# leo19941227/Speech-Enhancement-by-S3PRL

Hardware: AMD Instinct MI355X
Metric: enhanced 10s utts/sec (higher is better)
Workload: dtype bf16; 1 GPU; configs[1]: TERA/Mockingjay upstream (6x768x12x3072, pretrain_sample.yaml) + TransformerSpecPredictionHead, evaluate()-style pass, 10 s @ 16 kHz; batch_per_gpu=32, global_batch=32, layers=6, frames=1001, parallelism=dp1 (utterance-sharded inference, no data-path collective), weights=seeded random, real sizes, ranks=single process, no process group

## Files before the change

include/se_amd.h:

```cpp
#ifndef SE_AMD_H_
#define SE_AMD_H_

#include <stddef.h>
#include <stdint.h>

#ifdef __cplusplus
extern "C" {
#endif

typedef enum se_status {
  SE_OK = 0,
  SE_ERR_INVALID = -1,
  SE_ERR_UNSUPPORTED = -2,
  SE_ERR_HIP = -3,
  SE_ERR_OOM = -4,
  SE_ERR_NO_DEVICE = -5
} se_status;

typedef enum se_act { SE_ACT_IDENTITY = 0, SE_ACT_RELU = 1, SE_ACT_SIGMOID = 2, SE_ACT_GELU = 3, SE_ACT_EXP = 4 } se_act;

const char* se_last_error(void);
const char* se_version(void);
int se_device_available(void);

typedef struct se_plan se_plan;

typedef struct se_geometry {
  int sample_rate;
  int win;
  int hop;
  int n_freq;
  int n_mels;
} se_geometry;

int se_plan_create(const se_geometry* geom, se_plan** out);
int se_plan_create_any(const se_geometry* geom, se_plan** out);
void se_plan_destroy(se_plan* plan);
int se_plan_n_fft(const se_plan* plan);
int se_plan_chunk_frames(const se_plan* plan, int inverse);
int se_plan_tables(const se_plan* plan, float* window, float* mel_fb);

int se_num_frames(const se_plan* plan, int n_samples);

int se_stft_f32(const se_plan* plan, const float* wavs, int B, int C, int T, int channel,
                float* power, float* phase, float* complx, float* mel, void* stream);
int se_stft2_f32(const se_plan* plan, const float* wavs, int B, int C, int T, int channel_a, float* power_a, float* phase_a, float* complx_a,
                 float* mel_a, int channel_b, float* power_b, float* phase_b, float* complx_b, float* mel_b, void* stream);

int se_stft_tphase_f32(const se_plan* plan, const float* wavs, int B, int C, int T, int channel_a, float* power_a, unsigned* tphase_a, float* mel_a,
                       int channel_b, float* power_b, unsigned* tphase_b, float* mel_b, void* stream);

size_t se_features_workspace_bytes(int B, int D, int F, int delta);
int se_features_f32(const float* raw, int raw_time_major, int B, int D, int F,
                    int apply_log, int delta, int cmvn, float eps,
                    float* out, void* workspace, size_t workspace_bytes, void* stream);
int se_features2_f32(const float* raw, int raw_time_major, int B, int D, int F,
                     int apply_log, int delta, int cmvn, float eps,
                     float* out, void* workspace, size_t workspace_bytes,
                     uint16_t* out_bf16_pad, int ld_pad, int32_t* valid_count, void* stream);

size_t se_features3_workspace_bytes(int B, int D, int delta);
size_t se_features3_colstats_workspace_bytes(int B, int D, int F, int delta);
int se_features3_f32(const float* raw, int raw_time_major, int B, int D, int F, int apply_log, int delta, int cmvn, float eps,
                     float* out, void* workspace, size_t workspace_bytes, uint16_t* out_bf16_pad, int ld_pad, int32_t* valid_count,
                     float* colstats_out, float colstats_eps, void* stream);

int se_istft_f32(const se_plan* plan, const float* power, const float* phase, int B, int F,
                 float linear_power, float* wav_out, int wav_stride,
                 const int64_t* lengths, float* sumsq_out, void* stream);

int se_istft_tphase_f32(const se_plan* plan, const float* power, const unsigned* tphase, int B, int F, int log_input,
                        float* wav_out, int wav_stride, const int64_t* lengths, float* sumsq_out,
                        const float* ref, int ref_stride, float* ref_sumsq_out, void* stream);

int se_masked_sumsq_f32(const float* x, int B, int T, int x_stride, const int64_t* lengths, float* sums, void* stream);

int se_dbnorm_f32(float* wav, int B, int T, int wav_stride, const int64_t* lengths,
                  const float* wav_sumsq, const float* ref_sumsq, float fixed_db, float eps, void* stream);

int se_dbnorm_bwd_f32(const float* wav_norm, const float* grad_out, int B, int T, int wav_stride, const int64_t* lengths,
                      const float* wav_sumsq, const float* ref_sumsq, float fixed_db, float eps, double* scratch, float* grad_wav,
                      void* stream);

int se_istft_bwd_f32(const se_plan* plan, const float* grad_wav, int wav_stride, const float* power, const float* phase,
                     const unsigned* tphase, int B, int F, float* grad_power, void* stream);
int se_istft_bwd_chunk_frames(const se_plan* plan);

size_t se_stft_bwd_workspace_bytes(const se_plan* plan, int B, int T);
int se_stft_bwd_f32(const se_plan* plan, const float* grad_power, const float* grad_complx, const float* complx, int B, int F, int T,
                    float* grad_wav, int wav_stride, void* workspace, size_t workspace_bytes, void* stream);
int se_stft_bwd_chunk(const se_plan* plan);

int se_length_masks_i64(const int64_t* lengths, int B, int max_len, int64_t* masks, void* stream);

size_t se_head_workspace_bytes(int B, int F, int D, int N);
int se_head_linear_f32(const float* feats, const float* W, const float* bias, const float* linears,
                       int B, int F, int D, int N, int act, int cmvn, float eps,
                       float* predicted, float* offset, void* workspace, size_t workspace_bytes, void* stream);

size_t se_head_w3_bytes(int N, int D);
int se_head_colstats_f32(const float* feats, int B, int F, int D, float eps, float* stats, void* stream);
int se_head_split_weights_f32(const float* W, int N, int D, uint16_t* W3, void* stream);
int se_head_linear_pre_f32(const float* feats, const uint16_t* W3, const float* bias, const float* linears, const float* stats,
                           int B, int F, int D, int N, int act, float* predicted, float* offset, void* stream);

size_t se_head_sisdr_scratch_doubles(int B, int F, int N);
int se_head_linear_sisdr_f32(const float* feats, const uint16_t* W3, const float* bias, const float* linears, const float* stats,
                             int B, int F, int D, int N, int act, float* predicted, float* offset,
                             const float* linear_tar, const int64_t* lengths, int len_div, float eps, double* scratch,
                             float* loss_b, double* sums_out, float* loss_out, void* stream);
int se_sisdr_head_mean_f32(const double* slab, int B, int F, int tile_rows, float eps, float* loss_b, double* sums_out, float* loss_out, void* stream);

int se_head_linear_bwd_f32(const float* feats, const float* linears, const float* offset, const float* grad_predicted,
                           const float* grad_offset, int B, int F, int D, int N, int act, int cmvn, float eps,
                           float* gW, float* gb, void* workspace, size_t workspace_bytes, void* stream);
size_t se_head_dx_workspace_bytes(int B, int F, int D, int N);
int se_head_linear_dx_f32(const float* feats, const float* linears, const float* offset, const float* grad_predicted,
                          const float* grad_offset, const float* W, int B, int F, int D, int N, int act, int cmvn, float eps,
                          float* dx, void* workspace, size_t workspace_bytes, void* stream);

int se_l1_masked_f32(const float* log_pred, const float* linear_tar, const int64_t* frame_lengths,
                     int B, int F, int K, float eps, double* sums, float* grad, void* stream);
size_t se_l1_scratch_doubles(int B);
int se_l1_masked_loss_f32(const float* log_pred, const float* linear_tar, const int64_t* lengths, int len_div, int B, int F, int K, float eps,
                          double* scratch3, double* sums_out, float* loss_out, float* grad, void* stream);

typedef struct se_encoder se_encoder;

typedef struct se_encoder_config {
  int input_dim;
  int hidden;
  int layers;
  int heads;
  int intermediate;
  float ln_eps;
  int spec_out;
  int fused_ln_min_rows;
} se_encoder_config;

typedef struct se_encoder_weights {
  const float *in_w, *in_b, *in_ln_w, *in_ln_b;
  const float* const *q_w, * const *q_b, * const *k_w, * const *k_b, * const *v_w, * const *v_b;
  const float* const *ao_w, * const *ao_b, * const *aln_w, * const *aln_b;
  const float* const *ff1_w, * const *ff1_b, * const *ff2_w, * const *ff2_b, * const *oln_w, * const *oln_b;
  const float *sh_dense_w, *sh_dense_b, *sh_ln_w, *sh_ln_b, *sh_out_w, *sh_out_b;
} se_encoder_weights;

int se_encoder_create(const se_encoder_config* cfg, const se_encoder_weights* w, se_encoder** out);
void se_encoder_destroy(se_encoder* enc);
size_t se_encoder_workspace_bytes(const se_encoder* enc, int B, int T);

int se_encoder_fwd_bf16(const se_encoder* enc, const float* feats, const int32_t* lengths, int B, int T,
                        float* hidden, void* workspace, size_t workspace_bytes, void* stream);
int se_encoder_fwd2_bf16(const se_encoder* enc, const float* feats, const uint16_t* feats_bf16_pad, const int32_t* lengths, int B, int T,
                         float* hidden, void* workspace, size_t workspace_bytes, void* stream);

int se_spechead_fwd_bf16(const se_encoder* enc, const float* hidden, int B, int T, int log_target, int act, float eps,
                         float* predicted, float* log_predicted, float* raw,
                         void* workspace, size_t workspace_bytes, void* stream);
int se_spechead_fwd2_bf16(const se_encoder* enc, const float* hidden, int B, int T, int log_target, int act, float eps,
                          float* predicted, float* log_predicted, float* raw,
                          void* workspace, size_t workspace_bytes, int x_bf_valid, void* stream);

int se_valid_lengths_i32(const float* feats, int B, int T, int D, int32_t* lengths, void* stream);

int se_gemm_bf16(const uint16_t* A, int lda, const uint16_t* W, int ldw, const float* bias,
                 const float* residual_f32, int M, int N, int K, int act,
                 uint16_t* out_bf16, float* out_f32, int ldc, void* stream);
int se_gemm_res_ln_bf16(const uint16_t* A, int lda, const uint16_t* W, int ldw, const float* bias, const float* residual_f32,
                        const float* ln_w, const float* ln_b, float eps, int M, int N, int K,
                        float* out_f32, uint16_t* out_bf16, void* stream);
int se_mhsa_fwd_bf16(const uint16_t* qkv, const int32_t* lengths, int B, int T, int heads, uint16_t* ctx, void* stream);
int se_mhsa_fwd_prescaled_bf16(const uint16_t* qkv, const int32_t* lengths, int B, int T, int heads, uint16_t* ctx, void* stream);
int se_mhsa_fwd_prescaled_variant_bf16(const uint16_t* qkv, const int32_t* lengths, int B, int T, int heads, uint16_t* ctx, int variant, void* stream);
size_t se_gemm_res24_scratch_bytes(void);
size_t se_gemm_res24_lo_bytes(int M);
int se_gemm_res24_ln_bf16(const uint16_t* A, int lda, const uint16_t* W, int ldw, const float* bias, const uint16_t* res_hi, const uint8_t* res_lo,
                          const float* ln_w, const float* ln_b, float eps, int M, int N, int K, float* out_f32, uint16_t* out_bf16, uint8_t* out_lo,
                          int variant, void* scratch, void* stream);

int se_layernorm_f32(const float* x, const float* w, const float* b, int M, int H, float eps,
                     float* out_f32, uint16_t* out_bf16, void* stream);
int se_cast_f32_bf16(const float* x, size_t n, uint16_t* out, void* stream);

int se_gemm_f32(const float* A, long lda, const float* W, long ldw, int w_kmajor, const float* bias, const float* residual, int res_mod,
                int M, int N, int K, int act, float alpha, float* C, long ldc, int batch_outer, int batch_inner, long strideA_outer,
                long strideA_inner, long strideW_outer, long strideW_inner, long strideC_outer, long strideC_inner, void* stream);
int se_softmax_rows_f32(float* scores, const int32_t* lengths, int B, int heads, int T, void* stream);
int se_split3_bf16(const float* x, long ld, int rows, int cols, int Kp, int which, uint16_t* out, void* stream);

int se_gemm_x3out_bf16(const uint16_t* A, int lda, const uint16_t* W, int ldw, const float* bias, int M, int N, int K, int act,
                       uint16_t* out3, int Kp, void* stream);
int se_layernorm_x3_f32(const float* x, const float* w, const float* b, int M, int H, float eps, float* out_f32, uint16_t* out3, int Kp,
                        void* stream);
int se_mhsa_fwd_x3_split_f32(const float* qkv, const int32_t* lengths, int B, int T, int heads, uint16_t* ctx3, int Kp, void* stream);
int se_gemm_res_ln_x3_bf16(const uint16_t* A, int lda, const uint16_t* W, int ldw, const float* bias, const float* residual_f32, const float* ln_w,
                           const float* ln_b, float eps, int M, int N, int K, float* out_f32, uint16_t* out3, void* stream);
int se_mhsa_fwd_x3_f32(const float* qkv, const int32_t* lengths, int B, int T, int heads, float* ctx, void* stream);

int se_transpose_bf16(const uint16_t* in, int rows, int cols, int ld_in, uint16_t* out, int ld_out, void* stream);
int se_transpose_f32_bf16(const float* in, int rows, int cols, int ld_in, uint16_t* out, int ld_out, void* stream);
int se_wgrad_bf16(const uint16_t* dYt, const uint16_t* Xt, int Mp, int N, int K, int splits, float* dW, int accumulate,
                  void* workspace, size_t workspace_bytes, void* stream);
int se_wgrad_tn_bf16(const uint16_t* dY, int ldy, const uint16_t* X, int ldx, int M, int N, int K, int splits, float* dW,
                     int accumulate, void* workspace, size_t workspace_bytes, void* stream);
int se_wgrad_tn_slabs_bf16(const uint16_t* dY, int ldy, const uint16_t* X, int ldx, int M, int N, int K, int rows_per_slab,
                           float* slabs, void* stream);
int se_colsum_f32(const float* x, int rows, int cols, int ld, float* out, int accumulate, void* stream);
int se_colsum_groups(const void* x, int is_bf16, int groups, int rows, int cols, int ld, float* out, void* stream);
int se_layernorm_bwd_f32(const float* x_in, const float* dy, const float* w, int M, int H, float eps, int gelu_in,
                         float* dx, uint16_t* dx_bf16, float* dgamma, float* dbeta, int accumulate, void* stream);
int se_layernorm_bwd_groups_f32(const float* x_in, const float* dy, const float* w, int groups, int rows, int H, float eps, int gelu_in,
                                float* dx, uint16_t* dx_bf16, float* dgamma, float* dbeta, void* stream);
int se_gelu_layernorm_f32(const float* pre, const float* w, const float* b, int M, int H, float eps,
                          float* out_f32, uint16_t* out_bf16, void* stream);
int se_spec_epilogue_f32(const float* p, size_t n, int log_target, int act, float eps, float* predicted, float* log_predicted, void* stream);
int se_spec_epilogue_bwd_f32(const float* p, const float* d_pred, const float* d_logp, int M, int N, int ldp, int log_target,
                             int act, float eps, float* dp_f32, uint16_t* dp_bf16, void* stream);

int se_mhsa_fwd_lse_bf16(const uint16_t* qkv, const int32_t* lengths, int B, int T, int heads, uint16_t* ctx, float* lse,
                         float dropout_p, uint64_t seed, uint32_t site, void* stream);
int se_mhsa_bwd_bf16(const uint16_t* qkv, const uint16_t* ctx, const uint16_t* d_ctx, const float* lse, const int32_t* lengths,
                     int B, int T, int heads, uint16_t* dqkv, float* dvec, float dropout_p, uint64_t seed, uint32_t site, void* stream);
int se_gelu_bf16(const uint16_t* x, size_t n, uint16_t* y, void* stream);
int se_gelu_bwd_bf16(const uint16_t* dy, const uint16_t* x, size_t n, uint16_t* dx, void* stream);

typedef struct se_encoder_grads {
  float *in_w, *in_b, *in_ln_w, *in_ln_b;
  float* const *q_w, * const *q_b, * const *k_w, * const *k_b, * const *v_w, * const *v_b;
  float* const *ao_w, * const *ao_b, * const *aln_w, * const *aln_b;
  float* const *ff1_w, * const *ff1_b, * const *ff2_w, * const *ff2_b, * const *oln_w, * const *oln_b;
} se_encoder_grads;

int se_encoder_refresh_bf16(se_encoder* enc, const se_encoder_weights* w, void* stream);
size_t se_encoder_saved_bytes(const se_encoder* enc, int B, int T);
size_t se_encoder_train_workspace_bytes(const se_encoder* enc, int B, int T);
int se_encoder_fwd_train_bf16(const se_encoder* enc, const float* feats, const int32_t* lengths, int B, int T, float* hidden,
                              void* saved, size_t saved_bytes, void* workspace, size_t workspace_bytes, float dropout_p, uint64_t seed,
                              void* stream);
int se_encoder_bwd_bf16(const se_encoder* enc, const int32_t* lengths, int B, int T, const float* d_hidden, const void* saved,
                        size_t saved_bytes, const se_encoder_grads* grads, void* workspace, size_t workspace_bytes, float dropout_p,
                        uint64_t seed, void* stream);
int se_encoder_bwd_cb_bf16(const se_encoder* enc, const int32_t* lengths, int B, int T, const float* d_hidden, const void* saved,
                           size_t saved_bytes, const se_encoder_grads* g, void* workspace, size_t workspace_bytes, float dropout_p,
                           uint64_t seed, void (*layer_done)(int layer, void* user), void* user, void* stream);

int se_multi_sumsq_f32(const float* const* grads, const uint64_t* sizes, int n_tensors, double* sumsq, void* stream);
int se_bertadam_step_f32(float* const* params, const float* const* grads, float* const* m, float* const* v, const uint64_t* sizes,
                         const float* weight_decay, int n_tensors, const double* sumsq, double lr_t, double b1, double b2, double e,
                         double max_grad_norm, double global_max_norm, void* stream);
int se_multi_copy_f32(float* const* dsts, const float* const* srcs, const uint64_t* sizes, int n_tensors, void* stream);

int se_mix_f32(const float* speech, int ld_s, const int64_t* len_s, const float* noise, int ld_n, const int64_t* len_n,
               const int64_t* off_n, const float* snr_db, int B, int T_out, int normalize, float target_level_db, float eps,
               float* wavs, double* sums, void* stream);
int se_sisdr_f32(const float* src, const float* tar, int ld, const int64_t* lengths, int B, float eps, double* sums, float* sisdr,
                 void* stream);
int se_sisdr_grad_f32(const float* src, const float* tar, int ld, const int64_t* lengths, int B, float eps, const double* sums,
                      float grad_scale, float* grad, void* stream);

typedef struct se_stoi_plan se_stoi_plan;
int se_stoi_plan_create(int sample_rate, se_stoi_plan** out);
void se_stoi_plan_destroy(se_stoi_plan* plan);
size_t se_stoi_workspace_bytes(const se_stoi_plan* plan, int B, int T);
int se_stoi_f32(const se_stoi_plan* plan, const float* clean, const float* processed, int ld, const int64_t* lengths, int B, int T, int extended,
                float* stoi_out, int32_t* kept_out, float* tob_out, void* workspace, size_t workspace_bytes, void* stream);
size_t se_stoi_grad_workspace_bytes(const se_stoi_plan* plan, int B, int T);
int se_stoi_grad_f32(const se_stoi_plan* plan, const float* clean, const float* processed, int ld, const int64_t* lengths, int B, int T,
                     int extended, float grad_scale, float* stoi_out, float* grad , void* workspace, size_t workspace_bytes,
                     void* stream);

int se_lstm_fwd_bf16(const uint16_t* w_hh, const float* xproj, int B, int T, int ndir, uint16_t* h_out, float* gates_out, float* c_out,
                     void* stream);
int se_lstm_bwd_bf16(const uint16_t* w_hh_t, const float* gates, const float* c_saved, const float* dh_out, int ld_dh, int B, int T,
                     int ndir, uint16_t* dgates_out, void* stream);
int se_colsum_bf16(const uint16_t* x, int rows, int cols, int ld, float* out, void* stream);

int se_sisdr_spec_f32(const float* predicted, const float* linear_tar, const int64_t* frame_lengths, int B, int F, int N, float eps,
                      float grad_scale, double* scratch, float* loss_b, float* grad, void* stream);

size_t se_sisdr_spec_loss_scratch_doubles(int B, int F, int N);
int se_sisdr_spec_loss_f32(const float* predicted, const float* linear_tar, const int64_t* lengths, int len_div, int B, int F, int N, float eps,
                           double* scratch, float* loss_b, double* sums_out, float* loss_out, void* stream);

int se_wsd_energy_f32(const float* linear_tar, int B, int F, int N, float* energy, float* energy_max, void* stream);
int se_wsd_f32(const float* linear_inp, const float* offset, const float* linear_tar, const int64_t* frame_lengths, const float* energy,
               const float* energy_max, int B, int F, int N, float alpha, float db_interval, float eps, float grad_scale, double* sums,
               float* grad, void* stream);

size_t se_specdist_scratch_doubles(int B, int F, int K);
int se_specdist_loss_f32(const float* power_pred, const float* power_tar, const int64_t* lengths, int hop, int B, int F, int K, float clamp,
                         double* scratch, float* loss_b, void* stream);
int se_specdist_grad_f32(const float* power_pred, const float* power_tar, const int64_t* lengths, int hop, int B, int F, int K, float clamp,
                         const double* scratch, float grad_scale, float* grad_power_pred, void* stream);

int se_prof_enable(int on);
int se_prof_reset(void);
int se_prof_read(int kind, double* total_ms, double* total_work, long long* launches);

#ifdef __cplusplus
}
#endif
#endif
```

speech-enhancement-by-s3prl_amd/_lib.py:

```python
import ctypes
import os
from ctypes import POINTER, c_char_p, c_double, c_float, c_int, c_int32, c_int64, c_size_t, c_uint16, c_void_p

import torch

from . import checkpoint as _checkpoint

_HERE = os.path.dirname(os.path.abspath(__file__))
LIB_PATH = os.environ.get('SE_AMD_LIB') or os.path.join(_HERE, 'libse_amd.so')

SE_ACT = {'Identity': 0, 'ReLU': 1, 'Sigmoid': 2, 'GELU': 3, 'Exp': 4}


class SEError(RuntimeError):
    pass


class Geometry(ctypes.Structure):
    _fields_ = [('sample_rate', c_int), ('win', c_int), ('hop', c_int), ('n_freq', c_int), ('n_mels', c_int)]


class EncoderConfig(ctypes.Structure):
    _fields_ = [('input_dim', c_int), ('hidden', c_int), ('layers', c_int), ('heads', c_int), ('intermediate', c_int),
                ('ln_eps', c_float), ('spec_out', c_int), ('fused_ln_min_rows', c_int)]


_FP = POINTER(c_float)
_FPP = POINTER(_FP)


class EncoderWeights(ctypes.Structure):
    _fields_ = ([(n, _FP) for n in ('in_w', 'in_b', 'in_ln_w', 'in_ln_b')] +
                [(n, _FPP) for n in ('q_w', 'q_b', 'k_w', 'k_b', 'v_w', 'v_b', 'ao_w', 'ao_b', 'aln_w', 'aln_b',
                                     'ff1_w', 'ff1_b', 'ff2_w', 'ff2_b', 'oln_w', 'oln_b')] +
                [(n, _FP) for n in ('sh_dense_w', 'sh_dense_b', 'sh_ln_w', 'sh_ln_b', 'sh_out_w', 'sh_out_b')])


class EncoderGrads(ctypes.Structure):
    _fields_ = ([(n, _FP) for n in ('in_w', 'in_b', 'in_ln_w', 'in_ln_b')] +
                [(n, _FPP) for n in ('q_w', 'q_b', 'k_w', 'k_b', 'v_w', 'v_b', 'ao_w', 'ao_b', 'aln_w', 'aln_b',
                                     'ff1_w', 'ff1_b', 'ff2_w', 'ff2_b', 'oln_w', 'oln_b')])


_P = c_void_p
LAYER_DONE_CB = ctypes.CFUNCTYPE(None, c_int, c_void_p)
SIGNATURES = {
    'se_last_error': (c_char_p, []),
    'se_version': (c_char_p, []),
    'se_device_available': (c_int, []),
    'se_plan_create': (c_int, [POINTER(Geometry), POINTER(_P)]),
    'se_plan_create_any': (c_int, [POINTER(Geometry), POINTER(_P)]),
    'se_plan_destroy': (None, [_P]),
    'se_plan_n_fft': (c_int, [_P]),
    'se_plan_chunk_frames': (c_int, [_P, c_int]),
    'se_plan_tables': (c_int, [_P, _P, _P]),
    'se_num_frames': (c_int, [_P, c_int]),
    'se_stft_f32': (c_int, [_P, _P, c_int, c_int, c_int, c_int, _P, _P, _P, _P, _P]),
    'se_stft2_f32': (c_int, [_P, _P, c_int, c_int, c_int, c_int, _P, _P, _P, _P, c_int, _P, _P, _P, _P, _P]),
    'se_stft_tphase_f32': (c_int, [_P, _P, c_int, c_int, c_int, c_int, _P, _P, _P, c_int, _P, _P, _P, _P]),
    'se_istft_tphase_f32': (c_int, [_P, _P, _P, c_int, c_int, c_int, _P, c_int, _P, _P, _P, c_int, _P, _P]),
    'se_features_workspace_bytes': (c_size_t, [c_int, c_int, c_int, c_int]),
    'se_features_f32': (c_int, [_P, c_int, c_int, c_int, c_int, c_int, c_int, c_int, c_float, _P, _P, c_size_t, _P]),
    'se_features2_f32': (c_int, [_P, c_int, c_int, c_int, c_int, c_int, c_int, c_int, c_float, _P, _P, c_size_t, _P, c_int, _P, _P]),
    'se_features3_workspace_bytes': (c_size_t, [c_int, c_int, c_int]),
    'se_features3_colstats_workspace_bytes': (c_size_t, [c_int, c_int, c_int, c_int]),
    'se_features3_f32': (c_int, [_P, c_int, c_int, c_int, c_int, c_int, c_int, c_int, c_float, _P, _P, c_size_t, _P, c_int, _P, _P, c_float, _P]),
    'se_istft_f32': (c_int, [_P, _P, _P, c_int, c_int, c_float, _P, c_int, _P, _P, _P]),
    'se_masked_sumsq_f32': (c_int, [_P, c_int, c_int, c_int, _P, _P, _P]),
    'se_dbnorm_f32': (c_int, [_P, c_int, c_int, c_int, _P, _P, _P, c_float, c_float, _P]),
    'se_dbnorm_bwd_f32': (c_int, [_P, _P, c_int, c_int, c_int, _P, _P, _P, c_float, c_float, _P, _P, _P]),
    'se_istft_bwd_f32': (c_int, [_P, _P, c_int, _P, _P, _P, c_int, c_int, _P, _P]),
    'se_istft_bwd_chunk_frames': (c_int, [_P]),
    'se_stft_bwd_workspace_bytes': (c_size_t, [_P, c_int, c_int]),
    'se_stft_bwd_f32': (c_int, [_P, _P, _P, _P, c_int, c_int, c_int, _P, c_int, _P, c_size_t, _P]),
    'se_stft_bwd_chunk': (c_int, [_P]),
    'se_length_masks_i64': (c_int, [_P, c_int, c_int, _P, _P]),
    'se_head_workspace_bytes': (c_size_t, [c_int, c_int, c_int, c_int]),
    'se_head_linear_f32': (c_int, [_P, _P, _P, _P, c_int, c_int, c_int, c_int, c_int, c_int, c_float, _P, _P, _P, c_size_t, _P]),
    'se_head_colstats_f32': (c_int, [_P, c_int, c_int, c_int, c_float, _P, _P]),
    'se_head_w3_bytes': (c_size_t, [c_int, c_int]),
    'se_head_split_weights_f32': (c_int, [_P, c_int, c_int, _P, _P]),
    'se_head_linear_pre_f32': (c_int, [_P, _P, _P, _P, _P, c_int, c_int, c_int, c_int, c_int, _P, _P, _P]),
    'se_head_sisdr_scratch_doubles': (c_size_t, [c_int, c_int, c_int]),
    'se_head_linear_sisdr_f32': (c_int, [_P, _P, _P, _P, _P, c_int, c_int, c_int, c_int, c_int, _P, _P, _P, _P, c_int, c_float, _P, _P, _P, _P, _P]),
    'se_sisdr_head_mean_f32': (c_int, [_P, c_int, c_int, c_int, c_float, _P, _P, _P, _P]),
    'se_head_linear_bwd_f32': (c_int, [_P, _P, _P, _P, _P, c_int, c_int, c_int, c_int, c_int, c_int, c_float, _P, _P, _P, c_size_t, _P]),
    'se_head_dx_workspace_bytes': (c_size_t, [c_int, c_int, c_int, c_int]),
    'se_head_linear_dx_f32': (c_int, [_P, _P, _P, _P, _P, _P, c_int, c_int, c_int, c_int, c_int, c_int, c_float, _P, _P, c_size_t, _P]),
    'se_l1_masked_f32': (c_int, [_P, _P, _P, c_int, c_int, c_int, c_float, _P, _P, _P]),
    'se_l1_scratch_doubles': (c_size_t, [c_int]),
    'se_l1_masked_loss_f32': (c_int, [_P, _P, _P, c_int, c_int, c_int, c_int, c_float, _P, _P, _P, _P, _P]),
    'se_encoder_create': (c_int, [POINTER(EncoderConfig), POINTER(EncoderWeights), POINTER(_P)]),
    'se_encoder_destroy': (None, [_P]),
    'se_encoder_workspace_bytes': (c_size_t, [_P, c_int, c_int]),
    'se_encoder_fwd_bf16': (c_int, [_P, _P, _P, c_int, c_int, _P, _P, c_size_t, _P]),
    'se_encoder_fwd2_bf16': (c_int, [_P, _P, _P, _P, c_int, c_int, _P, _P, c_size_t, _P]),
    'se_spechead_fwd_bf16': (c_int, [_P, _P, c_int, c_int, c_int, c_int, c_float, _P, _P, _P, _P, c_size_t, _P]),
    'se_spechead_fwd2_bf16': (c_int, [_P, _P, c_int, c_int, c_int, c_int, c_float, _P, _P, _P, _P, c_size_t, c_int, _P]),
    'se_valid_lengths_i32': (c_int, [_P, c_int, c_int, c_int, _P, _P]),
    'se_gemm_bf16': (c_int, [_P, c_int, _P, c_int, _P, _P, c_int, c_int, c_int, c_int, _P, _P, c_int, _P]),
    'se_gemm_res_ln_bf16': (c_int, [_P, c_int, _P, c_int, _P, _P, _P, _P, c_float, c_int, c_int, c_int, _P, _P, _P]),
    'se_gemm_res24_scratch_bytes': (c_size_t, []),
    'se_gemm_res24_lo_bytes': (c_size_t, [c_int]),
    'se_gemm_res24_ln_bf16': (c_int, [_P, c_int, _P, c_int, _P, _P, _P, _P, _P, c_float, c_int, c_int, c_int, _P, _P, _P, c_int, _P, _P]),
    'se_mhsa_fwd_bf16': (c_int, [_P, _P, c_int, c_int, c_int, _P, _P]),
    'se_mhsa_fwd_prescaled_bf16': (c_int, [_P, _P, c_int, c_int, c_int, _P, _P]),
    'se_mhsa_fwd_prescaled_variant_bf16': (c_int, [_P, _P, c_int, c_int, c_int, _P, c_int, _P]),
    'se_layernorm_f32': (c_int, [_P, _P, _P, c_int, c_int, c_float, _P, _P, _P]),
    'se_cast_f32_bf16': (c_int, [_P, c_size_t, _P, _P]),
    'se_gemm_f32': (c_int, [_P, ctypes.c_long, _P, ctypes.c_long, c_int, _P, _P, c_int, c_int, c_int, c_int, c_int, c_float, _P, ctypes.c_long, c_int, c_int,
                            ctypes.c_long, ctypes.c_long, ctypes.c_long, ctypes.c_long, ctypes.c_long, ctypes.c_long, _P]),
    'se_softmax_rows_f32': (c_int, [_P, _P, c_int, c_int, c_int, _P]),
    'se_split3_bf16': (c_int, [_P, ctypes.c_long, c_int, c_int, c_int, c_int, _P, _P]),
    'se_gemm_x3out_bf16': (c_int, [_P, c_int, _P, c_int, _P, c_int, c_int, c_int, c_int, _P, c_int, _P]),
    'se_layernorm_x3_f32': (c_int, [_P, _P, _P, c_int, c_int, c_float, _P, _P, c_int, _P]),
    'se_mhsa_fwd_x3_split_f32': (c_int, [_P, _P, c_int, c_int, c_int, _P, c_int, _P]),
    'se_gemm_res_ln_x3_bf16': (c_int, [_P, c_int, _P, c_int, _P, _P, _P, _P, c_float, c_int, c_int, c_int, _P, _P, _P]),
    'se_mhsa_fwd_x3_f32': (c_int, [_P, _P, c_int, c_int, c_int, _P, _P]),
    'se_transpose_bf16': (c_int, [_P, c_int, c_int, c_int, _P, c_int, _P]),
    'se_transpose_f32_bf16': (c_int, [_P, c_int, c_int, c_int, _P, c_int, _P]),
    'se_wgrad_bf16': (c_int, [_P, _P, c_int, c_int, c_int, c_int, _P, c_int, _P, c_size_t, _P]),
    'se_wgrad_tn_bf16': (c_int, [_P, c_int, _P, c_int, c_int, c_int, c_int, c_int, _P, c_int, _P, c_size_t, _P]),
    'se_wgrad_tn_slabs_bf16': (c_int, [_P, c_int, _P, c_int, c_int, c_int, c_int, c_int, _P, _P]),
    'se_colsum_f32': (c_int, [_P, c_int, c_int, c_int, _P, c_int, _P]),
    'se_colsum_groups': (c_int, [_P, c_int, c_int, c_int, c_int, c_int, _P, _P]),
    'se_layernorm_bwd_groups_f32': (c_int, [_P, _P, _P, c_int, c_int, c_int, c_float, c_int, _P, _P, _P, _P, _P]),
    'se_layernorm_bwd_f32': (c_int, [_P, _P, _P, c_int, c_int, c_float, c_int, _P, _P, _P, _P, c_int, _P]),
    'se_gelu_layernorm_f32': (c_int, [_P, _P, _P, c_int, c_int, c_float, _P, _P, _P]),
    'se_spec_epilogue_f32': (c_int, [_P, c_size_t, c_int, c_int, c_float, _P, _P, _P]),
    'se_spec_epilogue_bwd_f32': (c_int, [_P, _P, _P, c_int, c_int, c_int, c_int, c_int, c_float, _P, _P, _P]),
    'se_mhsa_fwd_lse_bf16': (c_int, [_P, _P, c_int, c_int, c_int, _P, _P, c_float, ctypes.c_uint64, ctypes.c_uint32, _P]),
    'se_mhsa_bwd_bf16': (c_int, [_P, _P, _P, _P, _P, c_int, c_int, c_int, _P, _P, c_float, ctypes.c_uint64, ctypes.c_uint32, _P]),
    'se_gelu_bf16': (c_int, [_P, c_size_t, _P, _P]),
    'se_gelu_bwd_bf16': (c_int, [_P, _P, c_size_t, _P, _P]),
    'se_encoder_refresh_bf16': (c_int, [_P, POINTER(EncoderWeights), _P]),
    'se_encoder_saved_bytes': (c_size_t, [_P, c_int, c_int]),
    'se_encoder_train_workspace_bytes': (c_size_t, [_P, c_int, c_int]),
    'se_encoder_fwd_train_bf16': (c_int, [_P, _P, _P, c_int, c_int, _P, _P, c_size_t, _P, c_size_t, c_float, ctypes.c_uint64, _P]),
    'se_encoder_bwd_bf16': (c_int, [_P, _P, c_int, c_int, _P, _P, c_size_t, POINTER(EncoderGrads), _P, c_size_t, c_float, ctypes.c_uint64, _P]),
    'se_encoder_bwd_cb_bf16': (c_int, [_P, _P, c_int, c_int, _P, _P, c_size_t, POINTER(EncoderGrads), _P, c_size_t, c_float, ctypes.c_uint64, _P, _P, _P]),
    'se_multi_sumsq_f32': (c_int, [_P, _P, c_int, _P, _P]),
    'se_bertadam_step_f32': (c_int, [_P, _P, _P, _P, _P, _P, c_int, _P, c_double, c_double, c_double, c_double, c_double, c_double, _P]),
    'se_multi_copy_f32': (c_int, [_P, _P, _P, c_int, _P]),
    'se_mix_f32': (c_int, [_P, c_int, _P, _P, c_int, _P, _P, _P, c_int, c_int, c_int, c_float, c_float, _P, _P, _P]),
    'se_sisdr_f32': (c_int, [_P, _P, c_int, _P, c_int, c_float, _P, _P, _P]),
    'se_sisdr_grad_f32': (c_int, [_P, _P, c_int, _P, c_int, c_float, _P, c_float, _P, _P]),
    'se_stoi_plan_create': (c_int, [c_int, POINTER(_P)]),
    'se_stoi_plan_destroy': (None, [_P]),
    'se_stoi_workspace_bytes': (c_size_t, [_P, c_int, c_int]),
    'se_stoi_f32': (c_int, [_P, _P, _P, c_int, _P, c_int, c_int, c_int, _P, _P, _P, _P, c_size_t, _P]),
    'se_stoi_grad_workspace_bytes': (c_size_t, [_P, c_int, c_int]),
    'se_stoi_grad_f32': (c_int, [_P, _P, _P, c_int, _P, c_int, c_int, c_int, c_float, _P, _P, _P, c_size_t, _P]),
    'se_lstm_fwd_bf16':(c_int, [_P, _P, c_int, c_int, c_int, _P, _P, _P, _P]),
    'se_lstm_bwd_bf16': (c_int, [_P, _P, _P, _P, c_int, c_int, c_int, c_int, _P, _P]),
    'se_colsum_bf16': (c_int, [_P, c_int, c_int, c_int, _P, _P]),
    'se_sisdr_spec_loss_scratch_doubles': (c_size_t, [c_int, c_int, c_int]),
    'se_sisdr_spec_loss_f32': (c_int, [_P, _P, _P, c_int, c_int, c_int, c_int, c_float, _P, _P, _P, _P, _P]),
    'se_sisdr_spec_f32': (c_int, [_P, _P, _P, c_int, c_int, c_int, c_float, c_float, _P, _P, _P, _P]),
    'se_wsd_energy_f32': (c_int, [_P, c_int, c_int, c_int, _P, _P, _P]),
    'se_wsd_f32': (c_int, [_P, _P, _P, _P, _P, _P, c_int, c_int, c_int, c_float, c_float, c_float, c_float, _P, _P, _P]),
    'se_specdist_scratch_doubles': (c_size_t, [c_int, c_int, c_int]),
    'se_specdist_loss_f32': (c_int, [_P, _P, _P, c_int, c_int, c_int, c_int, c_float, _P, _P, _P]),
    'se_specdist_grad_f32': (c_int, [_P, _P, _P, c_int, c_int, c_int, c_int, c_float, _P, c_float, _P, _P]),
    'se_prof_enable': (c_int, [c_int]),
    'se_prof_reset': (c_int, []),
    'se_prof_read': (c_int, [c_int, POINTER(c_double), POINTER(c_double), POINTER(ctypes.c_longlong)]),
}

_lib = None


def load():
    global _lib
    if _lib is not None:
        return _lib
    if not os.path.exists(LIB_PATH):
        raise SEError(f'{LIB_PATH} is missing: build it with `python speech-enhancement-by-s3prl_amd/build.py` '
                      '(or __graft_entry__.build()); the MI355X path has no CPU fallback')
    lib = ctypes.CDLL(LIB_PATH)
    for name, (res, args) in SIGNATURES.items():
        if not hasattr(lib, name) and os.environ.get('SE_AMD_ALLOW_PARTIAL') == '1':
            continue
        fn = getattr(lib, name)
        fn.restype = res
        fn.argtypes = args
    _lib = lib
    return lib


def last_error():
    return load().se_last_error().decode()


def check(status, what):
    if status != 0:
        raise SEError(f'{what} failed with status {status}: {last_error()}')


def ptr(t):
    if t is None:
        return None
    mat = getattr(t, 'materialize', None)
    if mat is not None:
        t = mat()
    if not t.is_cuda:
        raise SEError('libse_amd kernels take device tensors only (got a CPU tensor); there is no CPU fallback')
    if not t.is_contiguous():
        raise SEError('libse_amd kernels take contiguous tensors')
    return t.data_ptr()


def stream():
    return torch.cuda.current_stream().cuda_stream
```

speech-enhancement-by-s3prl_amd/csrc/encoder.hip:

```cpp
#include <math.h>
#include <stdlib.h>
#include <utility>
#include <vector>
#include "common.h"
#include "bf16.h"
#include "encoder_impl.h"

extern "C" int se_gemm2_splitk_launch(const uint16_t* A, int lda, const uint16_t* W, int ldw, int M, int N, int Kc, int splits,
                                      float* partials, void* stream);

namespace se {

template <int NV, int GELU_IN = 0>
__global__ __launch_bounds__(256) void layernorm_kernel(const float* __restrict__ x, const float* __restrict__ pe, int T,
                                                        const float* __restrict__ w, const float* __restrict__ b, int M, float eps,
                                                        float* __restrict__ out_f32, uint16_t* __restrict__ out_bf16) {
  constexpr int H = 256 * NV;
  const int lane = threadIdx.x & 63;
  const int row = blockIdx.x * 4 + (threadIdx.x >> 6);
  if (row >= M) return;
  const float* xr = x + (size_t)row * H;
  float4 v[NV];
#pragma unroll
  for (int i = 0; i < NV; ++i) v[i] = *reinterpret_cast<const float4*>(xr + (i * 64 + lane) * 4);
// ... 45 lines not shown
  const int lane = threadIdx.x & 63;
  const int row = blockIdx.x * 4 + (threadIdx.x >> 6);
  if (row >= M) return;
  float4 v[NV];
#pragma unroll
  for (int i = 0; i < NV; ++i) {
    const int c = (i * 64 + lane) * 4;
    const float4 bb = *reinterpret_cast<const float4*>(bias + c);
    const float4 rr = *reinterpret_cast<const float4*>(residual + (size_t)row * H + c);
    v[i] = make_float4(bb.x + rr.x, bb.y + rr.y, bb.z + rr.z, bb.w + rr.w);
    for (int sidx = 0; sidx < nslab; ++sidx) {
      const float4 p = *reinterpret_cast<const float4*>(partials + sidx * slab_stride + (size_t)row * H + c);
      v[i].x += p.x; v[i].y += p.y; v[i].z += p.z; v[i].w += p.w;
    }
  }
  float s = 0.f;
#pragma unroll
  for (int i = 0; i < NV; ++i) s += (v[i].x + v[i].y) + (v[i].z + v[i].w);
#pragma unroll
  for (int off = 32; off > 0; off >>= 1) s += __shfl_xor(s, off);
  const float mean = s * (1.0f / H);
  float q = 0.f;
#pragma unroll
  for (int i = 0; i < NV; ++i) {
    v[i].x -= mean; v[i].y -= mean; v[i].z -= mean; v[i].w -= mean;
    q += (v[i].x * v[i].x + v[i].y * v[i].y) + (v[i].z * v[i].z + v[i].w * v[i].w);
  }
#pragma unroll
  for (int off = 32; off > 0; off >>= 1) q += __shfl_xor(q, off);
  const float rstd = 1.0f / sqrtf(q * (1.0f / H) + eps);
#pragma unroll
  for (int i = 0; i < NV; ++i) {
    const int c = (i * 64 + lane) * 4;
    const float4 ww = *reinterpret_cast<const float4*>(w + c), bb = *reinterpret_cast<const float4*>(b + c);
    float4 y;
    y.x = ww.x * (v[i].x * rstd) + bb.x; y.y = ww.y * (v[i].y * rstd) + bb.y;
    y.z = ww.z * (v[i].z * rstd) + bb.z; y.w = ww.w * (v[i].w * rstd) + bb.w;
    if (out_f32) *reinterpret_cast<float4*>(out_f32 + (size_t)row * H + c) = y;
    if (out_bf16) *reinterpret_cast<uint2*>(out_bf16 + (size_t)row * H + c) = make_uint2(pack_bf16x2(y.x, y.y), pack_bf16x2(y.z, y.w));
  }
}

__global__ __launch_bounds__(256) void layernorm_generic_kernel(const float* __restrict__ x, const float* __restrict__ pe, int T,
                                                                const float* __restrict__ w, const float* __restrict__ b, int H, float eps,
                                                                float* __restrict__ out_f32, uint16_t* __restrict__ out_bf16) {
  __shared__ float red[4];
  const int row = blockIdx.x, tid = threadIdx.x;
  const float* xr = x + (size_t)row * H;
  const float* pr = pe ? pe + (size_t)(row % T) * H : nullptr;
  float s = 0.f;
  for (int c = tid; c < H; c += 256) s += xr[c] + (pr ? pr[c] : 0.f);
  for (int off = 32; off > 0; off >>= 1) s += __shfl_down(s, off);
  if ((tid & 63) == 0) red[tid >> 6] = s;
  __syncthreads();
  const float mean = (red[0] + red[1] + red[2] + red[3]) / (float)H;
  __syncthreads();
  float q = 0.f;
  for (int c = tid; c < H; c += 256) {
    const float d = xr[c] + (pr ? pr[c] : 0.f) - mean;
    q += d * d;
  }
  for (int off = 32; off > 0; off >>= 1) q += __shfl_down(q, off);
  if ((tid & 63) == 0) red[tid >> 6] = q;
  __syncthreads();
  const float rstd = 1.0f / sqrtf((red[0] + red[1] + red[2] + red[3]) / (float)H + eps);
  for (int c = tid; c < H; c += 256) {
    const float y = w[c] * ((xr[c] + (pr ? pr[c] : 0.f) - mean) * rstd) + b[c];
    if (out_f32) out_f32[(size_t)row * H + c] = y;
    if (out_bf16) out_bf16[(size_t)row * H + c] = f2bf(y);
  }
}

__global__ __launch_bounds__(256) void cast_pad_kernel(const float* __restrict__ x, size_t rows, int cols, int ld_out,
                                                       uint16_t* __restrict__ out) {
  const size_t n4 = rows * (size_t)(ld_out / 4);
  for (size_t i = blockIdx.x * (size_t)256 + threadIdx.x; i < n4; i += (size_t)gridDim.x * 256) {
    const size_t r = i / (ld_out / 4);
    const int c = (int)(i - r * (ld_out / 4)) * 4;
    float v0 = 0.f, v1 = 0.f, v2 = 0.f, v3 = 0.f;
    const float* xr = x + r * cols;
    if (c + 3 < cols && (cols % 4 == 0)) {
      const float4 t = *reinterpret_cast<const float4*>(xr + c);
      v0 = t.x; v1 = t.y; v2 = t.z; v3 = t.w;
    } else {
      if (c < cols) v0 = xr[c];
      if (c + 1 < cols) v1 = xr[c + 1];
      if (c + 2 < cols) v2 = xr[c + 2];
      if (c + 3 < cols) v3 = xr[c + 3];
    }
    *reinterpret_cast<uint2*>(out + r * ld_out + c) = make_uint2(pack_bf16x2(v0, v1), pack_bf16x2(v2, v3));
  }
}

__global__ __launch_bounds__(256) void valid_lengths_kernel(const float* __restrict__ feats, int T, int D, int32_t* __restrict__ lengths) {
  __shared__ int red[4];
  const int b = blockIdx.y, lane = threadIdx.x & 63, wv = threadIdx.x >> 6;
  int cnt = 0;
  for (int t = blockIdx.x * 4 + wv; t < T; t += gridDim.x * 4) {
    const float* fr = feats + ((size_t)b * T + t) * D;
    float s = 0.f;
    for (int d = lane; d < D; d += 64) s += fr[d];
#pragma unroll
    for (int off = 32; off > 0; off >>= 1) s += __shfl_xor(s, off);
    cnt += (s != 0.f) ? 1 : 0;
  }
  if (lane == 0) red[wv] = cnt;
  __syncthreads();
  if (threadIdx.x == 0) atomicAdd(&lengths[b], red[0] + red[1] + red[2] + red[3]);
}

__global__ __launch_bounds__(256) void spec_epilogue_kernel(const float* __restrict__ p, size_t n, int log_target, int act, float eps,
                                                            float* __restrict__ predicted, float* __restrict__ log_predicted) {
  for (size_t i = blockIdx.x * (size_t)256 + threadIdx.x; i < n; i += (size_t)gridDim.x * 256) {
    const float v = p[i];
    float pred, lp;
    if (log_target == 2) {
      lp = (act == SE_ACT_RELU) ? fmaxf(v, 0.f) : (act == SE_ACT_SIGMOID) ? 1.f / (1.f + expf(-v)) : v;
      pred = expf(lp);
    } else {
      if (log_target) {
        pred = expf(v);
        lp = v;
      } else {
        pred = v;
        lp = logf(v + eps);
      }
      if (act == SE_ACT_RELU) pred = fmaxf(pred, 0.f);
      else if (act == SE_ACT_SIGMOID) pred = 1.f / (1.f + expf(-pred));
    }
    if (predicted) predicted[i] = pred;
    if (log_predicted) log_predicted[i] = lp;
  }
}

__global__ __launch_bounds__(256) void spec_epilogue_rows_kernel(const float* __restrict__ p, int M, int N, int ld, int log_target, int act, float eps,
                                                                 float* __restrict__ predicted, float* __restrict__ log_predicted) {
  for (int r = blockIdx.x; r < M; r += gridDim.x) {
    for (int c = threadIdx.x; c < N; c += 256) {
      const float v = p[(size_t)r * ld + c];
      float pred, lp;
      if (log_target) {
        pred = expf(v);
        lp = v;
      } else {
        pred = v;
        lp = logf(v + eps);
      }
      if (act == SE_ACT_RELU) pred = fmaxf(pred, 0.f);
      else if (act == SE_ACT_SIGMOID) pred = 1.f / (1.f + expf(-pred));
      const size_t o = (size_t)r * N + c;
      if (predicted) predicted[o] = pred;
      if (log_predicted) log_predicted[o] = lp;
    }
  }
}

__global__ __launch_bounds__(256) void spec_epilogue_bwd_kernel(const float* __restrict__ p, const float* __restrict__ d_pred,
                                                                const float* __restrict__ d_logp, int M, int N, int ldp, int log_target,
                                                                int act, float eps, float* __restrict__ dp_f32, uint16_t* __restrict__ dp_bf16) {
  const size_t n = (size_t)M * ldp;
  for (size_t i = blockIdx.x * (size_t)256 + threadIdx.x; i < n; i += (size_t)gridDim.x * 256) {
    const size_t r = i / ldp;
    const int c = (int)(i - r * ldp);
    float g = 0.f;
    if (c < N) {
      const size_t j = r * N + c;
      const float v = p[j];
      const float gp = d_pred ? d_pred[j] : 0.f, gl = d_logp ? d_logp[j] : 0.f;
      if (log_target == 2) {
        const float sg = 1.f / (1.f + expf(-v));
        const float lp = (act == SE_ACT_RELU) ? fmaxf(v, 0.f) : (act == SE_ACT_SIGMOID) ? sg : v;
        const float da = (act == SE_ACT_RELU) ? (v > 0.f ? 1.f : 0.f) : (act == SE_ACT_SIGMOID) ? sg * (1.f - sg) : 1.f;
        g = (gl + gp * expf(lp)) * da;
      } else if (log_target) {
        const float e = expf(v);
        const float da = (act == SE_ACT_RELU) ? (e > 0.f ? 1.f : 0.f) : 1.f;
        g = gl + gp * da * e;
      } else {
        const float da = (act == SE_ACT_RELU) ? (v > 0.f ? 1.f : 0.f) : 1.f;
        g = gp * da + gl / (v + eps);
      }
      if (dp_f32) dp_f32[j] = g;
    }
    if (dp_bf16) dp_bf16[i] = f2bf(g);
  }
}

}

namespace se {
__global__ __launch_bounds__(256) void qkv_inf_kernel(const float* __restrict__ q_w, const float* __restrict__ q_b, const uint16_t* __restrict__ qkv_w,
                                                      const float* __restrict__ qkv_b, int H, uint16_t* __restrict__ w_inf, float* __restrict__ b_inf) {
  const size_t hh = (size_t)H * H;
  for (size_t e = (size_t)blockIdx.x * 256 + threadIdx.x; e < 3 * hh; e += (size_t)gridDim.x * 256)
    w_inf[e] = e < hh ? f2bf(q_w[e] * kQScale) : qkv_w[e];
  for (int e = blockIdx.x * 256 + threadIdx.x; e < 3 * H; e += gridDim.x * 256) b_inf[e] = e < H ? q_b[e] * kQScale : qkv_b[e];
}
int launch_qkv_inf(const float* q_w, const float* q_b, const uint16_t* qkv_w, const float* qkv_b, int H, uint16_t* qkv_w_inf, float* qkv_b_inf, hipStream_t st) {
  hipLaunchKernelGGL(qkv_inf_kernel, dim3(512), dim3(256), 0, st, q_w, q_b, qkv_w, qkv_b, H, qkv_w_inf, qkv_b_inf);
  SE_LAUNCH_CHECK();
  return SE_OK;
}
}

static inline uint16_t host_f2bf(float f) {
  uint32_t u;
  memcpy(&u, &f, 4);
  if ((u & 0x7fffffffu) > 0x7f800000u) return (uint16_t)((u >> 16) | 0x40);
  return (uint16_t)((u + 0x7fffu + ((u >> 16) & 1u)) >> 16);
}

int se::launch_cast_pad(const float* x, size_t rows, int cols, int ld_out, uint16_t* out, hipStream_t st) {
  const int grid = (int)std::min<size_t>((rows * (size_t)(ld_out / 4) + 255) / 256, 8192);
  hipLaunchKernelGGL(se::cast_pad_kernel, dim3(grid), dim3(256), 0, st, x, rows, cols, ld_out, out);
  SE_LAUNCH_CHECK();
  return SE_OK;
}

int se::launch_layernorm(const float* x, const float* pe, int T, const float* w, const float* b, int M, int H, float eps,
                         float* out_f32, uint16_t* out_bf16, hipStream_t st) {
  if (H == 768) {
    hipLaunchKernelGGL((se::layernorm_kernel<3>), dim3((M + 3) / 4), dim3(256), 0, st, x, pe, T, w, b, M, eps, out_f32, out_bf16);
  } else if (H == 256) {
    hipLaunchKernelGGL((se::layernorm_kernel<1>), dim3((M + 3) / 4), dim3(256), 0, st, x, pe, T, w, b, M, eps, out_f32, out_bf16);
  } else if (H == 512) {
    hipLaunchKernelGGL((se::layernorm_kernel<2>), dim3((M + 3) / 4), dim3(256), 0, st, x, pe, T, w, b, M, eps, out_f32, out_bf16);
  } else if (H == 1024) {
    hipLaunchKernelGGL((se::layernorm_kernel<4>), dim3((M + 3) / 4), dim3(256), 0, st, x, pe, T, w, b, M, eps, out_f32, out_bf16);
  } else {
    hipLaunchKernelGGL(se::layernorm_generic_kernel, dim3(M), dim3(256), 0, st, x, pe, T, w, b, H, eps, out_f32, out_bf16);
  }
  SE_LAUNCH_CHECK();
  return SE_OK;
}

extern "C" int se_layernorm_f32(const float* x, const float* w, const float* b, int M, int H, float eps,
                                float* out_f32, uint16_t* out_bf16, void* stream) {
  SE_REQUIRE(x && w && b && (out_f32 || out_bf16) && M > 0 && H > 0, "se_layernorm_f32: bad argument");
  return se::launch_layernorm(x, nullptr, 1, w, b, M, H, eps, out_f32, out_bf16, se::as_stream(stream));
}

extern "C" int se_gelu_layernorm_f32(const float* pre, const float* w, const float* b, int M, int H, float eps,
                                     float* out_f32, uint16_t* out_bf16, void* stream) {
  SE_REQUIRE(pre && w && b && (out_f32 || out_bf16) && M > 0, "se_gelu_layernorm_f32: bad argument");
  SE_REQUIRE(H == 768 || H == 256, "se_gelu_layernorm_f32: only H = 768 / 256 are built (got %d)", H);
  if (H == 768)
    hipLaunchKernelGGL((se::layernorm_kernel<3, 1>), dim3((M + 3) / 4), dim3(256), 0, se::as_stream(stream), pre, nullptr, 1, w, b, M, eps, out_f32, out_bf16);
  else
    hipLaunchKernelGGL((se::layernorm_kernel<1, 1>), dim3((M + 3) / 4), dim3(256), 0, se::as_stream(stream), pre, nullptr, 1, w, b, M, eps, out_f32, out_bf16);
  SE_LAUNCH_CHECK();
  return SE_OK;
}

extern "C" int se_spec_epilogue_f32(const float* p, size_t n, int log_target, int act, float eps, float* predicted, float* log_predicted,
                                    void* stream) {
  SE_REQUIRE(p && n > 0 && (predicted || log_predicted), "se_spec_epilogue_f32: bad argument");
  const int grid = (int)std::min<size_t>((n + 255) / 256, 8192);
  hipLaunchKernelGGL(se::spec_epilogue_kernel, dim3(grid), dim3(256), 0, se::as_stream(stream), p, n, log_target, act, eps, predicted, log_predicted);
  SE_LAUNCH_CHECK();
  return SE_OK;
}

extern "C" int se_spec_epilogue_bwd_f32(const float* p, const float* d_pred, const float* d_logp, int M, int N, int ldp, int log_target,
                                        int act, float eps, float* dp_f32, uint16_t* dp_bf16, void* stream) {
  SE_REQUIRE(p && (d_pred || d_logp) && (dp_f32 || dp_bf16) && M > 0 && N > 0 && ldp >= N, "se_spec_epilogue_bwd_f32: bad argument");
  SE_REQUIRE(act == SE_ACT_RELU || act == SE_ACT_IDENTITY || (log_target == 2 && act == SE_ACT_SIGMOID),
             "se_spec_epilogue_bwd_f32: activation must be ReLU or Identity (Sigmoid only with log_target 2)");
  const size_t n = (size_t)M * ldp;
  const int grid = (int)std::min<size_t>((n + 255) / 256, 8192);
  hipLaunchKernelGGL(se::spec_epilogue_bwd_kernel, dim3(grid), dim3(256), 0, se::as_stream(stream), p, d_pred, d_logp, M, N, ldp, log_target,
                     act, eps, dp_f32, dp_bf16);
  SE_LAUNCH_CHECK();
  return SE_OK;
}

extern "C" int se_cast_f32_bf16(const float* x, size_t n, uint16_t* out, void* stream) {
  SE_REQUIRE(x && out && n > 0 && n % 4 == 0, "se_cast_f32_bf16: n must be a positive multiple of 4");
  const size_t rows = n / 4;
  const int grid = (int)std::min<size_t>((rows + 255) / 256, 4096);
  hipLaunchKernelGGL(se::cast_pad_kernel, dim3(grid), dim3(256), 0, se::as_stream(stream), x, rows, 4, 4, out);
  SE_LAUNCH_CHECK();
  return SE_OK;
}

extern "C" int se_valid_lengths_i32(const float* feats, int B, int T, int D, int32_t* lengths, void* stream) {
  SE_REQUIRE(feats && lengths && B > 0 && T > 0 && D > 0, "se_valid_lengths_i32: bad argument");
  { const int zrc_ = se::zero_async(lengths, sizeof(int32_t) * B, se::as_stream(stream)); if (zrc_) return zrc_; }
  hipLaunchKernelGGL(se::valid_lengths_kernel, dim3(std::min(32, (T + 3) / 4), B), dim3(256), 0, se::as_stream(stream), feats, T, D, lengths);
  SE_LAUNCH_CHECK();
  return SE_OK;
}

extern "C" int se_encoder_create(const se_encoder_config* cfg, const se_encoder_weights* w, se_encoder** out) {
  SE_REQUIRE(cfg && w && out, "se_encoder_create: null argument");
  const int H = cfg->hidden, I = cfg->intermediate, L = cfg->layers, D = cfg->input_dim;
  if (cfg->heads <= 0 || H != cfg->heads * 64 || H % 64 != 0 || I % 64 != 0 || D <= 0 || D > se::kInPad || L <= 0) {
    se::set_error("se_encoder_create: unsupported config (hidden=%d heads=%d intermediate=%d input_dim=%d): head dim must be 64, "
                  "hidden/intermediate multiples of 64, input_dim <= %d", H, cfg->heads, I, D, se::kInPad);
    return SE_ERR_UNSUPPORTED;
  }
  int ndev = 0;
  if (hipGetDeviceCount(&ndev) != hipSuccess || ndev <= 0) {
    (void)hipGetLastError();
    se::set_error("se_encoder_create: no HIP device visible (no CPU fallback)");
    return SE_ERR_NO_DEVICE;
  }
  const bool has_head = cfg->spec_out > 0 && w->sh_dense_w;
  std::vector<char> host;
  auto reserve = [&](size_t bytes) {
    const size_t off = (host.size() + 255) & ~(size_t)255;
    host.resize(off + bytes, 0);
    return off;
  };
  auto put_f32 = [&](const float* src, size_t n) {
    const size_t off = reserve(n * 4);
    memcpy(host.data() + off, src, n * 4);
    return off;
  };
  auto put_bf16 = [&](const float* src, int rows, int cols, int ld) {
    const size_t off = reserve((size_t)rows * ld * 2);
    uint16_t* d = reinterpret_cast<uint16_t*>(host.data() + off);
    for (int r = 0; r < rows; ++r)
      for (int c = 0; c < cols; ++c) d[(size_t)r * ld + c] = host_f2bf(src[(size_t)r * cols + c]);
    return off;
  };
  struct Off { size_t in_w, in_b, in_ln_w, in_ln_b, pe; std::vector<std::vector<size_t>> l; size_t shd_w, shd_b, shl_w, shl_b, sho_w, sho_b; } o;
  o.in_w = put_bf16(w->in_w, H, D, se::kInPad);
  o.in_b = put_f32(w->in_b, H);
  o.in_ln_w = put_f32(w->in_ln_w, H);
  o.in_ln_b = put_f32(w->in_ln_b, H);
  {
    o.pe = reserve((size_t)se::kMaxPos * H * 4);
    float* pe = reinterpret_cast<float*>(host.data() + o.pe);
    for (int pos = 0; pos < se::kMaxPos; ++pos)
      for (int j = 0; j < H; ++j) {
        const double ang = (double)pos / pow(10000.0, 2.0 * (double)(j / 2) / (double)H);
        pe[(size_t)pos * H + j] = (float)((j & 1) ? cos(ang) : sin(ang));
      }
  }
  for (int i = 0; i < L; ++i) {
    std::vector<size_t> lo;
    {
      const size_t off = reserve((size_t)3 * H * H * 2);
      uint16_t* d = reinterpret_cast<uint16_t*>(host.data() + off);
      const float* srcs[3] = {w->q_w[i], w->k_w[i], w->v_w[i]};
      for (int p = 0; p < 3; ++p)
        for (size_t e = 0; e < (size_t)H * H; ++e) d[(size_t)p * H * H + e] = host_f2bf(srcs[p][e]);
      lo.push_back(off);
      const size_t boff = reserve((size_t)3 * H * 4);
      float* bd = reinterpret_cast<float*>(host.data() + boff);
      memcpy(bd, w->q_b[i], H * 4);
      memcpy(bd + H, w->k_b[i], H * 4);
      memcpy(bd + 2 * H, w->v_b[i], H * 4);
      lo.push_back(boff);
    }
    size_t inf_w, inf_b;
    {
      inf_w = reserve((size_t)3 * H * H * 2);
      uint16_t* d = reinterpret_cast<uint16_t*>(host.data() + inf_w);
      for (size_t e = 0; e < (size_t)H * H; ++e) d[e] = host_f2bf(w->q_w[i][e] * se::kQScale);
      for (size_t e = 0; e < (size_t)H * H; ++e) d[(size_t)H * H + e] = host_f2bf(w->k_w[i][e]);
      for (size_t e = 0; e < (size_t)H * H; ++e) d[(size_t)2 * H * H + e] = host_f2bf(w->v_w[i][e]);
      inf_b = reserve((size_t)3 * H * 4);
      float* bd = reinterpret_cast<float*>(host.data() + inf_b);
      for (int e = 0; e < H; ++e) bd[e] = w->q_b[i][e] * se::kQScale;
      memcpy(bd + H, w->k_b[i], H * 4);
      memcpy(bd + 2 * H, w->v_b[i], H * 4);
    }
    lo.push_back(put_bf16(w->ao_w[i], H, H, H));
    lo.push_back(put_f32(w->ao_b[i], H));
    lo.push_back(put_f32(w->aln_w[i], H));
    lo.push_back(put_f32(w->aln_b[i], H));
    lo.push_back(put_bf16(w->ff1_w[i], I, H, H));
    lo.push_back(put_f32(w->ff1_b[i], I));
    lo.push_back(put_bf16(w->ff2_w[i], H, I, I));
    lo.push_back(put_f32(w->ff2_b[i], H));
    lo.push_back(put_f32(w->oln_w[i], H));
    lo.push_back(put_f32(w->oln_b[i], H));
    lo.push_back(inf_w);
    lo.push_back(inf_b);
    o.l.push_back(lo);
  }
  if (has_head) {
    o.shd_w = put_bf16(w->sh_dense_w, H, H, H);
    o.shd_b = put_f32(w->sh_dense_b, H);
    o.shl_w = put_f32(w->sh_ln_w, H);
    o.shl_b = put_f32(w->sh_ln_b, H);
    o.sho_w = put_bf16(w->sh_out_w, cfg->spec_out, H, H);
    reserve((size_t)3 * H * 2);
    o.sho_b = put_f32(w->sh_out_b, cfg->spec_out);
    reserve(3 * 4);
  }
  se_encoder* e = new se_encoder();
  e->cfg = *cfg;
  if (!has_head) e->cfg.spec_out = 0;
  e->blob_bytes = host.size() + 256;
  hipError_t err = hipMalloc(&e->blob, e->blob_bytes);
  if (err != hipSuccess) {
    delete e;
    return se::hip_fail(err, "hipMalloc(encoder weights)", __FILE__, __LINE__);
  }
  err = hipMemcpy(e->blob, host.data(), host.size(), hipMemcpyHostToDevice);
  if (err != hipSuccess) {
    (void)hipFree(e->blob);
    delete e;
    return se::hip_fail(err, "hipMemcpy(encoder weights)", __FILE__, __LINE__);
  }
  char* base = reinterpret_cast<char*>(e->blob);
  e->in_w = (uint16_t*)(base + o.in_w);
  e->in_b = (float*)(base + o.in_b);
  e->in_ln_w = (float*)(base + o.in_ln_w);
// ... 3 lines not shown
    const auto& lo = o.l[i];
    se_encoder::Layer y;
    y.qkv_w = (uint16_t*)(base + lo[0]); y.qkv_b = (float*)(base + lo[1]);
    y.ao_w = (uint16_t*)(base + lo[2]); y.ao_b = (float*)(base + lo[3]);
    y.aln_w = (float*)(base + lo[4]); y.aln_b = (float*)(base + lo[5]);
    y.ff1_w = (uint16_t*)(base + lo[6]); y.ff1_b = (float*)(base + lo[7]);
    y.ff2_w = (uint16_t*)(base + lo[8]); y.ff2_b = (float*)(base + lo[9]);
    y.oln_w = (float*)(base + lo[10]); y.oln_b = (float*)(base + lo[11]);
    y.qkv_w_inf = (uint16_t*)(base + lo[12]); y.qkv_b_inf = (float*)(base + lo[13]);
    e->layers.push_back(y);
  }
  if (has_head) {
    e->sh_dense_w = (uint16_t*)(base + o.shd_w); e->sh_dense_b = (float*)(base + o.shd_b);
    e->sh_ln_w = (float*)(base + o.shl_w); e->sh_ln_b = (float*)(base + o.shl_b);
    e->sh_out_w = (uint16_t*)(base + o.sho_w); e->sh_out_b = (float*)(base + o.sho_b);
  }
  *out = e;
  return SE_OK;
}

extern "C" void se_encoder_destroy(se_encoder* enc) {
  if (!enc) return;
  if (enc->blob) (void)hipFree(enc->blob);
  delete enc;
}

namespace {
struct Ws {
  uint16_t *xin, *x_bf, *qkv, *ctx, *h;
  float *x_f32, *tmp, *slabs;
  uint8_t* lo;
  char* g8;
  size_t total;
};
constexpr size_t kSplitKRows = 3072;
constexpr int kSplitK = 4;
using se::al256;
Ws carve(const se_encoder* e, size_t M, char* base) {
  const size_t H = e->cfg.hidden, I = e->cfg.intermediate;
  Ws w;
  size_t off = 0;
  auto take = [&](size_t bytes) { char* p = base ? base + off : nullptr; off += al256(bytes); return p; };
  w.xin = (uint16_t*)take(M * se::kInPad * 2);
  w.x_bf = (uint16_t*)take(M * H * 2);
  w.x_f32 = (float*)take(M * H * 4);
  w.tmp = (float*)take(M * H * 4);
  w.qkv = (uint16_t*)take(M * 3 * H * 2);
  w.ctx = (uint16_t*)take(M * H * 2);
  w.h = (uint16_t*)take(M * I * 2);
  w.slabs = (float*)take(M <= kSplitKRows ? (size_t)kSplitK * M * H * 4 : 0);
  w.lo = (uint8_t*)take(H == 768 ? se::gemm4_lo_bytes((int)M) : 0);
  w.g8 = take(H == 768 ? se::gemm8_scratch_bytes() : 0);
  w.total = off;
  return w;
}
}

extern "C" size_t se_encoder_workspace_bytes(const se_encoder* enc, int B, int T) {
  if (!enc || B <= 0 || T <= 0) return 0;
  return carve(enc, (size_t)B * T, nullptr).total + 256;
}

extern "C" int se_encoder_fwd_bf16(const se_encoder* enc, const float* feats, const int32_t* lengths, int B, int T,
                                   float* hidden, void* workspace, size_t workspace_bytes, void* stream) {
  return se_encoder_fwd2_bf16(enc, feats, nullptr, lengths, B, T, hidden, workspace, workspace_bytes, stream);
}

extern "C" int se_encoder_fwd2_bf16(const se_encoder* enc, const float* feats, const uint16_t* feats_bf16_pad, const int32_t* lengths, int B, int T,
                                    float* hidden, void* workspace, size_t workspace_bytes, void* stream) {
  SE_REQUIRE(enc && (feats || feats_bf16_pad) && hidden && workspace, "se_encoder_fwd_bf16: null argument");
  SE_REQUIRE((uintptr_t)feats_bf16_pad % 16 == 0, "se_encoder_fwd2_bf16: the bf16 feature rows must be 16-B aligned");
  SE_REQUIRE(B > 0 && B <= 65535 && T > 0 && T <= se::kMaxPos, "se_encoder_fwd_bf16: bad shape B=%d T=%d (T <= %d)", B, T, se::kMaxPos);
  SE_REQUIRE(workspace_bytes >= se_encoder_workspace_bytes(enc, B, T), "se_encoder_fwd_bf16: workspace too small");
  SE_REQUIRE((uintptr_t)workspace % 256 == 0 && (uintptr_t)hidden % 16 == 0, "se_encoder_fwd_bf16: workspace must be 256-B aligned");
  const int H = enc->cfg.hidden, I = enc->cfg.intermediate, D = enc->cfg.input_dim;
  const size_t Mz = (size_t)B * T;
  SE_REQUIRE(Mz <= 0x7fffffff / 4, "se_encoder_fwd_bf16: B*T too large");
  const int M = (int)Mz;
  hipStream_t st = se::as_stream(stream);
  Ws w = carve(enc, Mz, reinterpret_cast<char*>(workspace));
  int rc;
  if (feats_bf16_pad) {
    w.xin = const_cast<uint16_t*>(feats_bf16_pad);
  } else {
    const int grid = (int)std::min<size_t>((Mz * (se::kInPad / 4) + 255) / 256, 8192);
    hipLaunchKernelGGL(se::cast_pad_kernel, dim3(grid), dim3(256), 0, st, feats, Mz, D, se::kInPad, w.xin);
    SE_LAUNCH_CHECK();
  }
  const int L = enc->cfg.layers;
  static int fuse_env = -1;
  if (fuse_env < 0) {
    const char* e = getenv("SE_AMD_FUSED_LN");
    fuse_env = e ? atoi(e) : 1;
  }
  const bool fused = fuse_env && H == 768 && I % 32 == 0 && I >= 128 && (fuse_env == 2 || M >= (enc->cfg.fused_ln_min_rows > 0 ? enc->cfg.fused_ln_min_rows : 16000));
#ifdef SE_AMD_EXPERIMENTS
  static int use8 = -1;
  if (use8 < 0) { const char* e8 = getenv("SE_AMD_GEMM8"); use8 = e8 ? atoi(e8) : 0; }
  if (fused && use8) {
    const size_t fo = se::gemm8_scratch_bytes() - (128 * 2 * 4 + 256);
    if ((rc = se::zero_async(w.g8 + fo, 128 * 2 * 4 + 256, st))) return rc;
  }
#endif
  if (fused) {
    if ((rc = se::launch_gemm_pos_ln(w.xin, se::kInPad, enc->in_w, se::kInPad, enc->in_b, enc->pe, T, enc->in_ln_w, enc->in_ln_b, enc->cfg.ln_eps, M, H,
                                     se::kInPad, nullptr, w.x_bf, w.lo, st))) return rc;
  } else {
    if ((rc = se_gemm_bf16(w.xin, se::kInPad, enc->in_w, se::kInPad, enc->in_b, nullptr, M, H, se::kInPad, SE_ACT_IDENTITY, nullptr, w.tmp, H, stream))) return rc;
    if ((rc = se::launch_layernorm(w.tmp, enc->pe, T, enc->in_ln_w, enc->in_ln_b, M, H, enc->cfg.ln_eps, w.x_f32, w.x_bf, st))) return rc;
  }
  for (int i = 0; i < L; ++i) {
    const se_encoder::Layer& y = enc->layers[i];
    if ((rc = se_gemm_bf16(w.x_bf, H, y.qkv_w_inf, H, y.qkv_b_inf, nullptr, M, 3 * H, H, SE_ACT_IDENTITY, w.qkv, nullptr, 3 * H, stream))) return rc;
    if ((rc = se_mhsa_fwd_prescaled_bf16(w.qkv, lengths, B, T, enc->cfg.heads, w.ctx, stream))) return rc;
    if (fused) {
      if ((rc = se::launch_gemm_res24_ln(w.ctx, H, y.ao_w, H, y.ao_b, w.x_bf, w.lo, y.aln_w, y.aln_b, enc->cfg.ln_eps, M, H, H, nullptr, w.x_bf, w.lo, st))) return rc;
    } else {
      if ((rc = se_gemm_bf16(w.ctx, H, y.ao_w, H, y.ao_b, w.x_f32, M, H, H, SE_ACT_IDENTITY, nullptr, w.tmp, H, stream))) return rc;
      if ((rc = se::launch_layernorm(w.tmp, nullptr, 1, y.aln_w, y.aln_b, M, H, enc->cfg.ln_eps, w.x_f32, w.x_bf, st))) return rc;
    }
    if ((rc = se_gemm_bf16(w.x_bf, H, y.ff1_w, H, y.ff1_b, nullptr, M, I, H, SE_ACT_GELU, w.h, nullptr, I, stream))) return rc;
    if (fused) {
      float* of = (i == L - 1) ? hidden : nullptr;
      uint16_t* ob = w.x_bf;
      uint8_t* ol = (i == L - 1) ? nullptr : w.lo;
      rc = 1;
#ifdef SE_AMD_EXPERIMENTS
      rc = se::launch_gemm8_res24_ln(w.h, I, y.ff2_w, I, y.ff2_b, w.x_bf, w.lo, y.oln_w, y.oln_b, enc->cfg.ln_eps, M, H, I, of, ob, ol, w.g8, st);
#endif
      if (rc == 1) rc = se::launch_gemm_res24_ln(w.h, I, y.ff2_w, I, y.ff2_b, w.x_bf, w.lo, y.oln_w, y.oln_b, enc->cfg.ln_eps, M, H, I, of, ob, ol, st);
      if (rc) return rc;
    } else {
      float* xo = (i == L - 1) ? hidden : w.x_f32;
      if (Mz <= kSplitKRows && H == 768 && I % (kSplitK * 64) == 0 && I / kSplitK >= 128) {
        if ((rc = se_gemm2_splitk_launch(w.h, I, y.ff2_w, I, M, H, I / kSplitK, kSplitK, w.slabs, stream))) return rc;
        hipLaunchKernelGGL((se::ln_reduce_kernel<3>), dim3((M + 3) / 4), dim3(256), 0, st, w.slabs, kSplitK, Mz * H, y.ff2_b, w.x_f32, y.oln_w, y.oln_b, M,
                           enc->cfg.ln_eps, xo, w.x_bf);
        SE_LAUNCH_CHECK();
      } else {
        if ((rc = se_gemm_bf16(w.h, I, y.ff2_w, I, y.ff2_b, w.x_f32, M, H, I, SE_ACT_IDENTITY, nullptr, w.tmp, H, stream))) return rc;
        if ((rc = se::launch_layernorm(w.tmp, nullptr, 1, y.oln_w, y.oln_b, M, H, enc->cfg.ln_eps, xo, w.x_bf, st))) return rc;
      }
    }
  }
  return SE_OK;
}

extern "C" int se_spechead_fwd_bf16(const se_encoder* enc, const float* hidden, int B, int T, int log_target, int act, float eps,
                                    float* predicted, float* log_predicted, float* raw,
                                    void* workspace, size_t workspace_bytes, void* stream) {
  return se_spechead_fwd2_bf16(enc, hidden, B, T, log_target, act, eps, predicted, log_predicted, raw, workspace, workspace_bytes, 0, stream);
}

extern "C" int se_spechead_fwd2_bf16(const se_encoder* enc, const float* hidden, int B, int T, int log_target, int act, float eps,
                                     float* predicted, float* log_predicted, float* raw,
                                     void* workspace, size_t workspace_bytes, int x_bf_valid, void* stream) {
  SE_REQUIRE(enc && hidden && workspace && (predicted || log_predicted || raw), "se_spechead_fwd_bf16: null argument");
  SE_REQUIRE(enc->cfg.spec_out > 0, "se_spechead_fwd_bf16: encoder was created without a spec head");
  SE_REQUIRE(B > 0 && T > 0, "se_spechead_fwd_bf16: bad shape");
  SE_REQUIRE(workspace_bytes >= se_encoder_workspace_bytes(enc, B, T), "se_spechead_fwd_bf16: workspace too small");
  const int H = enc->cfg.hidden, N = enc->cfg.spec_out;
  const size_t Mz = (size_t)B * T;
  const int M = (int)Mz;
  hipStream_t st = se::as_stream(stream);
  Ws w = carve(enc, Mz, reinterpret_cast<char*>(workspace));
  int rc;
  if (!x_bf_valid) {
    const int grid = (int)std::min<size_t>((Mz * (H / 4) + 255) / 256, 8192);
    hipLaunchKernelGGL(se::cast_pad_kernel, dim3(grid), dim3(256), 0, st, hidden, Mz, H, H, w.x_bf);
    SE_LAUNCH_CHECK();
  }
  static int fuse_env = -1;
  if (fuse_env < 0) {
    const char* e = getenv("SE_AMD_FUSED_LN");
    fuse_env = e ? atoi(e) : 1;
  }
  if (fuse_env && H == 768 && (fuse_env == 2 || M >= (enc->cfg.fused_ln_min_rows > 0 ? enc->cfg.fused_ln_min_rows : 16000))) {
    if ((rc = se::launch_gemm_gelu_ln(w.x_bf, H, enc->sh_dense_w, H, enc->sh_dense_b, enc->sh_ln_w, enc->sh_ln_b, enc->cfg.ln_eps, M, H, H, nullptr,
                                      w.ctx, st))) return rc;
  } else {
    if ((rc = se_gemm_bf16(w.x_bf, H, enc->sh_dense_w, H, enc->sh_dense_b, nullptr, M, H, H, SE_ACT_GELU, nullptr, w.tmp, H, stream))) return rc;
    if ((rc = se::launch_layernorm(w.tmp, nullptr, 1, enc->sh_ln_w, enc->sh_ln_b, M, H, enc->cfg.ln_eps, nullptr, w.ctx, st))) return rc;
  }
  float* p = raw ? raw : w.x_f32;
  const int Np = raw ? N : (N + 3) & ~3;
  const int ldp = raw ? N : (N + 7) & ~7;
  SE_REQUIRE(ldp <= H, "se_spechead_fwd_bf16: spec_out %d exceeds the hidden size %d", N, H);
  if ((rc = se_gemm_bf16(w.ctx, H, enc->sh_out_w, H, enc->sh_out_b, nullptr, M, Np, H, SE_ACT_IDENTITY, nullptr, p, ldp, stream))) return rc;
  if (predicted || log_predicted) {
    hipLaunchKernelGGL(se::spec_epilogue_rows_kernel, dim3(std::min(M, 8192)), dim3(256), 0, st, p, M, N, ldp, log_target, act, eps, predicted,
                       log_predicted);
    SE_LAUNCH_CHECK();
  }
  return SE_OK;
}
```

speech-enhancement-by-s3prl_amd/csrc/istft.hip:

```cpp
#include <stdlib.h>
#include "plan.h"
#include "prof.h"
#include "fft200.h"

namespace se {

#ifndef SE_ISTFT_FR
#define SE_ISTFT_FR 30
#endif
constexpr int kIFR = SE_ISTFT_FR;
constexpr int kIHB = kIFR - 3;
constexpr int kISpan = kIHB * kHop;
constexpr int kIThreads = 256;
constexpr int kIPairs = 101;
constexpr int kIPairIters = (kIFR * kIPairs + kIThreads - 1) / kIThreads;
constexpr int kIRefIters = (kISpan / 4 + kIThreads - 1) / kIThreads;
constexpr float kIScale = 1.0f / 400.0f;

template <int SQRT, int ENC>
__global__ __launch_bounds__(kIThreads) void istft_kernel(
    const float* __restrict__ power, const float* __restrict__ phase, int F, float inv_lp,
    const float* __restrict__ window, const float2* __restrict__ tw400g, const float2* __restrict__ tw200g,
    float* __restrict__ wav, int wav_stride, const int64_t* __restrict__ lengths, float* __restrict__ sumsq,
    const float* __restrict__ ref, int ref_stride, float* __restrict__ ref_sumsq) {
// ... 148 lines not shown
    } else {
      wrow[n] = v.x; wrow[n + 1] = v.y; wrow[n + 2] = v.z; wrow[n + 3] = v.w;
    }
    if (n < len_b) ss = fmaf(v.x, v.x, ss);
    if (n + 1 < len_b) ss = fmaf(v.y, v.y, ss);
    if (n + 2 < len_b) ss = fmaf(v.z, v.z, ss);
    if (n + 3 < len_b) ss = fmaf(v.w, v.w, ss);
  }
  if (blockIdx.x == gridDim.x - 1)
    for (int n = n_out + tid; n < wav_stride; n += kIThreads) wav[(size_t)b * wav_stride + n] = 0.f;

  if (sumsq) {
    float sr = rtail;
    if (ref_sumsq) {
#pragma unroll
      for (int i = 0; i < kIRefIters; ++i) sr += rq[i][0] * rq[i][0] + rq[i][1] * rq[i][1] + rq[i][2] * rq[i][2] + rq[i][3] * rq[i][3];
    }
#pragma unroll
    for (int off = 32; off > 0; off >>= 1) {
      ss += __shfl_down(ss, off);
      sr += __shfl_down(sr, off);
    }
    if ((tid & 63) == 0) { red[0][tid >> 6] = ss; red[1][tid >> 6] = sr; }
    __syncthreads();
    if (tid == 0) atomicAdd(&sumsq[b], red[0][0] + red[0][1] + red[0][2] + red[0][3]);
    if (tid == 64 && ref_sumsq) atomicAdd(&ref_sumsq[b], red[1][0] + red[1][1] + red[1][2] + red[1][3]);
  }
}

__global__ __launch_bounds__(256) void masked_sumsq_kernel(const float* __restrict__ x, int T, int x_stride,
                                                           const int64_t* __restrict__ lengths, float* __restrict__ sums) {
  __shared__ float red[4];
  const int b = blockIdx.y;
  const int len = (int)min((int64_t)T, max((int64_t)0, lengths[b]));
  const float* row = x + (size_t)b * x_stride;
  float ss = 0.f;
  if ((reinterpret_cast<uintptr_t>(row) & 15) == 0) {
    const int len4 = len >> 2, stride = gridDim.x * 256;
    float4 acc = make_float4(0.f, 0.f, 0.f, 0.f);
    for (int n = blockIdx.x * 256 + threadIdx.x; n < len4; n += 2 * stride) {
      const float4 a = reinterpret_cast<const float4*>(row)[n];
      const float4 c = (n + stride < len4) ? reinterpret_cast<const float4*>(row)[n + stride] : make_float4(0.f, 0.f, 0.f, 0.f);
      acc.x = fmaf(a.x, a.x, fmaf(c.x, c.x, acc.x));
      acc.y = fmaf(a.y, a.y, fmaf(c.y, c.y, acc.y));
      acc.z = fmaf(a.z, a.z, fmaf(c.z, c.z, acc.z));
      acc.w = fmaf(a.w, a.w, fmaf(c.w, c.w, acc.w));
    }
    ss = (acc.x + acc.y) + (acc.z + acc.w);
    if (blockIdx.x == 0 && threadIdx.x < (len & 3)) {
      const float v = row[4 * len4 + threadIdx.x];
      ss = fmaf(v, v, ss);
    }
  } else {
    for (int n = blockIdx.x * 256 + threadIdx.x; n < len; n += gridDim.x * 256) {
      const float v = row[n];
      ss = fmaf(v, v, ss);
    }
  }
#pragma unroll
  for (int off = 32; off > 0; off >>= 1) ss += __shfl_down(ss, off);
  if ((threadIdx.x & 63) == 0) red[threadIdx.x >> 6] = ss;
  __syncthreads();
  if (threadIdx.x == 0) atomicAdd(&sums[b], red[0] + red[1] + red[2] + red[3]);
}

__global__ __launch_bounds__(256) void dbnorm_kernel(float* __restrict__ wav, int T, int wav_stride,
                                                     const int64_t* __restrict__ lengths, const float* __restrict__ wav_sumsq,
                                                     const float* __restrict__ ref_sumsq, float fixed_db, float eps) {
  const int b = blockIdx.y;
  const float cnt = (float)min((int64_t)T, max((int64_t)0, lengths[b]));
  const float denom = cnt + eps;
  const float target_db = ref_sumsq ? 10.0f * log10f(ref_sumsq[b] / denom) : fixed_db;
  const float scale = sqrtf(powf(10.0f, target_db / 10.0f) / (wav_sumsq[b] / denom + eps));
  float* row = wav + (size_t)b * wav_stride;
  for (int n = blockIdx.x * 256 + threadIdx.x; n < T; n += gridDim.x * 256) row[n] *= scale;
}

__global__ __launch_bounds__(256) void dbnorm_bwd_dot_kernel(const float* __restrict__ y, const float* __restrict__ g, int T, int wav_stride,
                                                             double* __restrict__ dot) {
  __shared__ double red[4];
  const int b = blockIdx.y;
  const float* yr = y + (size_t)b * wav_stride;
  const float* gr = g + (size_t)b * wav_stride;
  double acc = 0.0;
  for (int n = blockIdx.x * 256 + threadIdx.x; n < T; n += gridDim.x * 256) acc += (double)yr[n] * (double)gr[n];
#pragma unroll
  for (int off = 32; off > 0; off >>= 1) acc += __shfl_down(acc, off);
  if ((threadIdx.x & 63) == 0) red[threadIdx.x >> 6] = acc;
  __syncthreads();
  if (threadIdx.x == 0) atomicAdd(&dot[b], (red[0] + red[1]) + (red[2] + red[3]));
}

__global__ __launch_bounds__(256) void dbnorm_bwd_apply_kernel(const float* __restrict__ y, const float* g, int T, int wav_stride,
                                                               const int64_t* __restrict__ lengths, const float* __restrict__ wav_sumsq,
                                                               const float* __restrict__ ref_sumsq, float fixed_db, float eps,
                                                               const double* __restrict__ dot, float* grad_wav) {
  const int b = blockIdx.y;
  const int len = (int)min((int64_t)T, max((int64_t)0, lengths[b]));
  const double denom = (double)((float)len + eps);
  const double R = ref_sumsq ? (double)ref_sumsq[b] / denom : pow(10.0, (double)fixed_db / 10.0);
  const double M = (double)wav_sumsq[b] / denom + (double)eps;
  const double sc = sqrt(R / M);
  const float scale = (float)sc;
  const float coef = sc > 0.0 ? (float)(dot[b] / (sc * M * denom)) : 0.f;
  const float* yr = y + (size_t)b * wav_stride;
  const float* gr = g + (size_t)b * wav_stride;
  float* o = grad_wav + (size_t)b * wav_stride;
  for (int n = blockIdx.x * 256 + threadIdx.x; n < T; n += gridDim.x * 256) {
    const float gv = gr[n], yv = yr[n];
    o[n] = (n < len) ? fmaf(-yv, coef, scale * gv) : scale * gv;
  }
}

__global__ void length_masks_kernel(const int64_t* __restrict__ lengths, int max_len, int64_t* __restrict__ masks) {
  const int b = blockIdx.y;
  const int64_t len = lengths[b];
  for (int t = blockIdx.x * blockDim.x + threadIdx.x; t < max_len; t += gridDim.x * blockDim.x)
    masks[(size_t)b * max_len + t] = (t < len) ? 1 : 0;
}

}

extern "C" int se_istft_f32(const se_plan* plan, const float* power, const float* phase, int B, int F,
                            float linear_power, float* wav_out, int wav_stride,
                            const int64_t* lengths, float* sumsq_out, void* stream) {
  SE_REQUIRE(plan && power && phase && wav_out, "se_istft_f32: null argument");
  SE_REQUIRE(B > 0 && B <= 65535 && F >= 2, "se_istft_f32: bad B=%d F=%d", B, F);
  const int n_out = plan->geom.hop * (F - 1);
  SE_REQUIRE(wav_stride >= n_out, "se_istft_f32: wav_stride=%d < %d output samples", wav_stride, n_out);
  SE_REQUIRE(linear_power > 0.f, "se_istft_f32: linear_power must be positive");
  SE_REQUIRE(sumsq_out == nullptr || lengths != nullptr, "se_istft_f32: sumsq_out needs lengths");
  if (plan->general)
    return se_istftg_launch(plan, power, phase, 0, 0, linear_power, B, F, wav_out, wav_stride, lengths, sumsq_out, nullptr, 0, nullptr, stream);
  hipStream_t st = se::as_stream(stream);
  if (sumsq_out) { const int zrc_ = se::zero_async(sumsq_out, sizeof(float) * B, st); if (zrc_) return zrc_; }
  dim3 grid((n_out + se::kISpan - 1) / se::kISpan, B);
  se::ProfScope prof(se::kProfIstft, (double)B * (8.0 * F * se::kBins + 4.0 * n_out), st);
  if (linear_power == 2.0f)
    hipLaunchKernelGGL((se::istft_kernel<1, 0>), grid, dim3(se::kIThreads), 0, st, power, phase, F, 0.5f, plan->d_window, plan->d_tw400, plan->d_tw200,
                       wav_out, wav_stride, lengths, sumsq_out, nullptr, 0, nullptr);
  else
    hipLaunchKernelGGL((se::istft_kernel<0, 0>), grid, dim3(se::kIThreads), 0, st, power, phase, F, 1.0f / linear_power, plan->d_window, plan->d_tw400,
                       plan->d_tw200, wav_out, wav_stride, lengths, sumsq_out, nullptr, 0, nullptr);
  SE_LAUNCH_CHECK();
  return SE_OK;
}

extern "C" int se_istft2p_tphase_f32(const se_plan* plan, const float* power, const unsigned* tphase, int B, int F, int log_input,
                                     float* wav_out, int wav_stride, const int64_t* lengths, float* sumsq_out, void* stream);

extern "C" int se_istft_tphase_f32(const se_plan* plan, const float* power, const unsigned* tphase, int B, int F, int log_input,
                                   float* wav_out, int wav_stride, const int64_t* lengths, float* sumsq_out,
                                   const float* ref, int ref_stride, float* ref_sumsq_out, void* stream) {
  SE_REQUIRE(plan && power && tphase && wav_out, "se_istft_tphase_f32: null argument");
  SE_REQUIRE(B > 0 && B <= 65535 && F >= 2, "se_istft_tphase_f32: bad B=%d F=%d", B, F);
  const int n_out = plan->geom.hop * (F - 1);
  SE_REQUIRE(wav_stride >= n_out, "se_istft_tphase_f32: wav_stride=%d < %d output samples", wav_stride, n_out);
  SE_REQUIRE(sumsq_out == nullptr || lengths != nullptr, "se_istft_tphase_f32: sumsq_out needs lengths");
  SE_REQUIRE(ref_sumsq_out == nullptr || (ref && sumsq_out && ref_stride >= n_out), "se_istft_tphase_f32: ref_sumsq_out needs ref (row stride >= %d) and sumsq_out", n_out);
  if (plan->general)
    return se_istftg_launch(plan, power, reinterpret_cast<const float*>(tphase), 1, log_input, 2.0f, B, F, wav_out, wav_stride, lengths, sumsq_out, ref,
                            ref_stride, ref_sumsq_out, stream);
#ifdef SE_AMD_EXPERIMENTS
  static const bool use2 = getenv("SE_AMD_STFT2") != nullptr;
#else
  const bool use2 = false;
#endif
  hipStream_t st = se::as_stream(stream);
  if (use2 || log_input) {
    int rc = se_istft2p_tphase_f32(plan, power, tphase, B, F, log_input, wav_out, wav_stride, lengths, sumsq_out, stream);
    if (rc == SE_OK && ref_sumsq_out) rc = se_masked_sumsq_f32(ref, B, std::min(wav_stride, ref_stride), ref_stride, lengths, ref_sumsq_out, stream);
    return rc;
  }
  if (sumsq_out) {
    int zrc_;
    if (ref_sumsq_out == sumsq_out + B) zrc_ = se::zero_async(sumsq_out, sizeof(float) * 2 * B, st);
    else {
      zrc_ = se::zero_async(sumsq_out, sizeof(float) * B, st);
      if (!zrc_ && ref_sumsq_out) zrc_ = se::zero_async(ref_sumsq_out, sizeof(float) * B, st);
    }
    if (zrc_) return zrc_;
  }
  dim3 grid((n_out + se::kISpan - 1) / se::kISpan, B);
  se::ProfScope prof(se::kProfIstft, (double)B * (8.0 * F * se::kBins + 4.0 * n_out), st);
  hipLaunchKernelGGL((se::istft_kernel<1, 1>), grid, dim3(se::kIThreads), 0, st, power, reinterpret_cast<const float*>(tphase), F, 0.5f, plan->d_window,
                     plan->d_tw400, plan->d_tw200, wav_out, wav_stride, lengths, sumsq_out, ref_sumsq_out ? ref : nullptr, ref_stride, ref_sumsq_out);
  SE_LAUNCH_CHECK();
  return SE_OK;
}

extern "C" int se_masked_sumsq_f32(const float* x, int B, int T, int x_stride, const int64_t* lengths, float* sums, void* stream) {
  SE_REQUIRE(x && lengths && sums && B > 0 && B <= 65535 && T > 0 && x_stride >= T, "se_masked_sumsq_f32: bad argument");
  hipStream_t st = se::as_stream(stream);
  { const int zrc_ = se::zero_async(sums, sizeof(float) * B, st); if (zrc_) return zrc_; }
  dim3 grid(std::min(32, (T + 2047) / 2048), B);
  hipLaunchKernelGGL(se::masked_sumsq_kernel, grid, dim3(256), 0, st, x, T, x_stride, lengths, sums);
  SE_LAUNCH_CHECK();
  return SE_OK;
}

extern "C" int se_dbnorm_f32(float* wav, int B, int T, int wav_stride, const int64_t* lengths,
                             const float* wav_sumsq, const float* ref_sumsq, float fixed_db, float eps, void* stream) {
  SE_REQUIRE(wav && lengths && wav_sumsq && B > 0 && B <= 65535 && T > 0 && wav_stride >= T, "se_dbnorm_f32: bad argument");
  dim3 grid(std::min(64, (T + 255) / 256), B);
  hipLaunchKernelGGL(se::dbnorm_kernel, grid, dim3(256), 0, se::as_stream(stream), wav, T, wav_stride, lengths, wav_sumsq,
                     ref_sumsq, fixed_db, eps);
  SE_LAUNCH_CHECK();
  return SE_OK;
}

extern "C" int se_dbnorm_bwd_f32(const float* wav_norm, const float* grad_out, int B, int T, int wav_stride, const int64_t* lengths,
                                 const float* wav_sumsq, const float* ref_sumsq, float fixed_db, float eps, double* scratch, float* grad_wav,
                                 void* stream) {
  SE_REQUIRE(wav_norm && grad_out && lengths && wav_sumsq && scratch && grad_wav && B > 0 && B <= 65535 && T > 0 && wav_stride >= T,
             "se_dbnorm_bwd_f32: bad argument");
  hipStream_t st = se::as_stream(stream);
  { const int zrc_ = se::zero_async(scratch, sizeof(double) * B, st); if (zrc_) return zrc_; }
  hipLaunchKernelGGL(se::dbnorm_bwd_dot_kernel, dim3(std::max(1, std::min(64, (T + 4095) / 4096)), B), dim3(256), 0, st, wav_norm, grad_out, T,
                     wav_stride, scratch);
  SE_LAUNCH_CHECK();
  hipLaunchKernelGGL(se::dbnorm_bwd_apply_kernel, dim3(std::min(64, (T + 255) / 256), B), dim3(256), 0, st, wav_norm, grad_out, T, wav_stride,
                     lengths, wav_sumsq, ref_sumsq, fixed_db, eps, scratch, grad_wav);
  SE_LAUNCH_CHECK();
  return SE_OK;
}

extern "C" int se_length_masks_i64(const int64_t* lengths, int B, int max_len, int64_t* masks, void* stream) {
  SE_REQUIRE(lengths && masks && B > 0 && B <= 65535 && max_len > 0, "se_length_masks_i64: bad argument");
  dim3 grid(std::min(256, (max_len + 255) / 256), B);
  hipLaunchKernelGGL(se::length_masks_kernel, grid, dim3(256), 0, se::as_stream(stream), lengths, max_len, masks);
  SE_LAUNCH_CHECK();
  return SE_OK;
}
```

speech-enhancement-by-s3prl_amd/decode.py:

```python
import torch

from . import _lib


def get_length_masks(lengths, max_len=None):
    lib = _lib.load()
    lengths = lengths.to(torch.int64).contiguous()
    if max_len is None:
        max_len = int(lengths.max().item())
    masks = torch.empty(lengths.shape[0], max_len, device=lengths.device, dtype=torch.int64)
    _lib.check(lib.se_length_masks_i64(_lib.ptr(lengths), lengths.shape[0], max_len, _lib.ptr(masks), _lib.stream()),
               'se_length_masks_i64')
    return masks


def masked_sumsq(x, lengths):
    lib = _lib.load()
    x = x.contiguous().float()
    B, T = x.shape
    lengths = lengths.to(device=x.device, dtype=torch.int64).contiguous()
    sums = torch.empty(B, device=x.device, dtype=torch.float32)
    _lib.check(lib.se_masked_sumsq_f32(_lib.ptr(x), B, T, T, _lib.ptr(lengths), _lib.ptr(sums), _lib.stream()), 'se_masked_sumsq_f32')
    return sums


class _DbNormFn(torch.autograd.Function):

    @staticmethod
    def forward(ctx, audio, target, lengths, eps, audio_sumsq, inplace, ref_sumsq):
        if inplace:
            ctx.mark_dirty(audio)
        ctx.args = []
        out = masked_normalize_decibel(audio, target, lengths, eps, audio_sumsq, inplace, ref_sumsq, _sums_out=ctx.args)
        lens, wav_sumsq, ref_sumsq, ctx.fixed = ctx.args
        ctx.eps, ctx.has_ref = float(eps), ref_sumsq is not None
        ctx.save_for_backward(out, lens, wav_sumsq, *([ref_sumsq] if ctx.has_ref else []))
        del ctx.args
        return out

    @staticmethod
    def backward(ctx, grad_out):
        lib = _lib.load()
        y, lens, wav_sumsq = ctx.saved_tensors[:3]
        ref_sumsq = ctx.saved_tensors[3] if ctx.has_ref else None
        B, T = y.shape
        g = grad_out.contiguous().float()
        grad_wav = torch.empty_like(g)
        scratch = torch.empty(B, device=y.device, dtype=torch.float64)
        _lib.check(lib.se_dbnorm_bwd_f32(_lib.ptr(y), _lib.ptr(g), B, T, T, _lib.ptr(lens), _lib.ptr(wav_sumsq), _lib.ptr(ref_sumsq), ctx.fixed, ctx.eps,
                                         _lib.ptr(scratch), _lib.ptr(grad_wav), _lib.stream()), 'se_dbnorm_bwd_f32')
        return grad_wav, None, None, None, None, None, None


def masked_normalize_decibel(audio, target, lengths, eps=1e-8, audio_sumsq=None, inplace=False, ref_sumsq=None, _sums_out=None):
    if torch.is_grad_enabled() and audio.requires_grad:
        if not audio.is_cuda:
            raise _lib.SEError('libse_amd kernels take device tensors only (got a CPU tensor); there is no CPU fallback')
        if audio.dtype != torch.float32 or not audio.is_contiguous():
            audio, inplace = audio.contiguous().float(), False
        return _DbNormFn.apply(audio, target, lengths, eps, audio_sumsq, inplace, ref_sumsq)
    lib = _lib.load()
    audio = audio.contiguous().float()
    if not inplace:
        audio = audio.clone()
    B, T = audio.shape
    lengths = lengths.to(device=audio.device, dtype=torch.int64).contiguous()
    if audio_sumsq is None:
        audio_sumsq = masked_sumsq(audio, lengths)
    fixed = 0.0
    if isinstance(target, (int, float)):
        fixed, ref_sumsq = float(target), None
    elif isinstance(target, torch.Tensor) and target.dim() > 1:
        if ref_sumsq is None:
            ref = target
            if ref.dtype != torch.float32 or ref.stride(1) != 1:
                ref = ref.contiguous().float()
            if ref.shape[1] < T:
                raise _lib.SEError('reference audio shorter than the audio to normalise')
            if not ref.is_cuda:
                raise _lib.SEError('reference audio must live on the GPU (no CPU fallback)')
            ref_sumsq = torch.empty(B, device=audio.device, dtype=torch.float32)
            _lib.check(lib.se_masked_sumsq_f32(ref.data_ptr(), B, T, ref.stride(0), _lib.ptr(lengths), _lib.ptr(ref_sumsq),
                                               _lib.stream()), 'se_masked_sumsq_f32')
    else:
        raise NotImplementedError('per-utterance dB tensor targets are unused by the reference')
    _lib.check(lib.se_dbnorm_f32(_lib.ptr(audio), B, T, T, _lib.ptr(lengths), _lib.ptr(audio_sumsq), _lib.ptr(ref_sumsq),
                                 fixed, float(eps), _lib.stream()), 'se_dbnorm_f32')
    if _sums_out is not None:
        _sums_out.extend([lengths, audio_sumsq, ref_sumsq, fixed])
    return audio


def decode_wav(preprocessor, linear, phase, lengths, target_level=-25, max_len=None):
    if max_len is None:
        max_len = int(lengths.max().item())
    ref = target_level if isinstance(target_level, torch.Tensor) and target_level.dim() == 2 else None
    if ref is not None:
        wav, sumsq, ref_sumsq = preprocessor.istft_with_sumsq(linear, phase, lengths=lengths, out_len=max_len, ref=ref)
        return masked_normalize_decibel(wav, target_level, lengths, audio_sumsq=sumsq, inplace=True, ref_sumsq=ref_sumsq)
    wav, sumsq = preprocessor.istft_with_sumsq(linear, phase, lengths=lengths, out_len=max_len)
    return masked_normalize_decibel(wav, target_level, lengths, audio_sumsq=sumsq, inplace=True)
```

speech-enhancement-by-s3prl_amd/heads.py:

```python
import torch
import torch.nn as nn

from . import _lib
from .checkpoint import load_checkpoint
from .preprocessor import OnlinePreprocessor
from .transformer import TRANSFORMER, TransformerConfig, TransformerSpecPredictionHead


class _HeadLinearFn(torch.autograd.Function):

    @staticmethod
    def forward(ctx, feats, linears, weight, bias, act, cmvn, eps):
        lib = _lib.load()
        B, F, D = feats.shape
        N = weight.shape[0]
        feats = feats.contiguous().float()
        lin = None if linears is None else linears.contiguous().float()
        w, b = weight.contiguous().float(), bias.contiguous().float()
        predicted = torch.empty(B, F, N, device=feats.device, dtype=torch.float32)
        offset = torch.empty(B, F, N, device=feats.device, dtype=torch.float32)
        nbytes = lib.se_head_workspace_bytes(B, F, D, N)
        ws = torch.empty(nbytes, device=feats.device, dtype=torch.uint8)
        _lib.check(lib.se_head_linear_f32(_lib.ptr(feats), _lib.ptr(w), _lib.ptr(b), _lib.ptr(lin), B, F, D, N, act,
                                          int(cmvn), float(eps), _lib.ptr(predicted), _lib.ptr(offset), _lib.ptr(ws), nbytes,
# ... 19 lines not shown
                                              B, F, D, N, act, cmvn, eps, _lib.ptr(gW), _lib.ptr(gb), _lib.ptr(ws), nbytes,
                                              _lib.stream()), 'se_head_linear_bwd_f32')
        d_feats = None
        if ctx.needs_input_grad[0]:
            d_feats = torch.empty_like(feats)
            nb = lib.se_head_dx_workspace_bytes(B, F, D, N)
            ws2 = torch.empty(nb, device=feats.device, dtype=torch.uint8)
            _lib.check(lib.se_head_linear_dx_f32(_lib.ptr(feats), _lib.ptr(lin) if has_lin else None, _lib.ptr(offset), _lib.ptr(gp), _lib.ptr(go),
                                                 _lib.ptr(w), B, F, D, N, act, cmvn, eps, _lib.ptr(d_feats), _lib.ptr(ws2), nb, _lib.stream()),
                       'se_head_linear_dx_f32')
        return d_feats, None, gW, gb, None, None, None


def _act_id(name):
    if name not in _lib.SE_ACT:
        raise NotImplementedError(f'activation nn.{name} is not supported by the HIP head kernel '
                                  f'(supported: {sorted(_lib.SE_ACT)})')
    return _lib.SE_ACT[name]


class Linear(nn.Module):

    def __init__(self, input_dim, output_dim, activation='ReLU', **kwargs):
        super().__init__()
        self.linear = nn.Linear(input_dim, output_dim)
        self.activation = activation
        self._act = _act_id(activation)

    def forward(self, features, **kwargs):
        predicted, _ = _HeadLinearFn.apply(features, None, self.linear.weight, self.linear.bias, self._act, False, 0.0)
        return predicted, {}


class LinearResidual(nn.Module):

    def __init__(self, input_size=201, output_size=201, activation='Sigmoid', cmvn=True, eps=1e-6, **kwargs):
        super().__init__()
        self.linear = nn.Linear(input_size, output_size)
        self.activation = activation
        self._act = _act_id(activation)
        self.cmvn = cmvn
        self.eps = eps

    def forward(self, features, linears, **kwargs):
        needs_grad = torch.is_grad_enabled() and (features.requires_grad or any(p.requires_grad for p in self.parameters()))
        if not needs_grad and features.is_cuda and getattr(self, 'lazy_offset', True):
            return self._forward_lazy(features, linears)
        predicted, offset = _HeadLinearFn.apply(features, linears, self.linear.weight, self.linear.bias, self._act,
                                                self.cmvn, self.eps)
        return predicted, {'offset': offset}

    def _w3(self, dev):
        import weakref
        w = self.linear.weight
        key = (w.data_ptr(), w._version, str(dev))
        c = getattr(self, '_w3_cache', None)
        if c is None or c[0] != key or c[2]() is not w:
            lib = _lib.load()
            N, D = w.shape
            wf = w.detach().contiguous().float()
            w3 = torch.empty(int(lib.se_head_w3_bytes(N, D)), device=dev, dtype=torch.uint8)
            _lib.check(lib.se_head_split_weights_f32(_lib.ptr(wf), N, D, _lib.ptr(w3), _lib.stream()), 'se_head_split_weights_f32')
            c = self._w3_cache = (key, w3, weakref.ref(w))
        return c[1]

    def _forward_lazy(self, features, linears, sisdr=None):
        from .preprocessor import LazyTensor
        lib = _lib.load()
        B, F, D = features.shape
        N = self.linear.weight.shape[0]
        feats = features.contiguous().float()
        lin = linears.contiguous().float()
        act, cmvn, eps = self._act, int(self.cmvn), float(self.eps)
        stats = None
        if cmvn:
            side = getattr(features, '_se_colstats', None)
            if side is not None and side[1] == eps and side[2] == features._version and feats.data_ptr() == features.data_ptr():
                stats = side[0]
            else:
                stats = torch.empty(B, D, 2, device=feats.device, dtype=torch.float32)
                _lib.check(lib.se_head_colstats_f32(_lib.ptr(feats), B, F, D, eps, _lib.ptr(stats), _lib.stream()), 'se_head_colstats_f32')
        w3 = self._w3(feats.device)
        bias = self.linear.bias.detach().contiguous().float()
        wkey = (self.linear.weight.data_ptr(), self.linear.weight._version, self.linear.bias._version)

        def run(want_offset):
            if (self.linear.weight.data_ptr(), self.linear.weight._version, self.linear.bias._version) != wkey:
                raise RuntimeError('LinearResidual: the parameters changed after forward() returned and before its lazy `offset` was read; read it first '
                                   '(or set head.lazy_offset = False)')
            out = torch.empty(B, F, N, device=feats.device, dtype=torch.float32)
            if want_offset:
                _lib.check(lib.se_head_linear_pre_f32(_lib.ptr(feats), _lib.ptr(w3), _lib.ptr(bias), None, _lib.ptr(stats), B, F, D, N, act, _lib.ptr(out), None,
                                                      _lib.stream()), 'se_head_linear_pre_f32')
            else:
                _lib.check(lib.se_head_linear_pre_f32(_lib.ptr(feats), _lib.ptr(w3), _lib.ptr(bias), _lib.ptr(lin), _lib.ptr(stats), B, F, D, N, act, _lib.ptr(out), None,
                                                      _lib.stream()), 'se_head_linear_pre_f32')
            return out
        if sisdr is not None:
            tar, lengths, len_div, ceps = sisdr
            tarc = tar.contiguous().float()
            lens = lengths.to(device=feats.device, dtype=torch.int64).contiguous()
            predicted = torch.empty(B, F, N, device=feats.device, dtype=torch.float32)
            scratch = torch.empty(int(lib.se_head_sisdr_scratch_doubles(B, F, N)) + 2, device=feats.device, dtype=torch.float64)
            loss_b = torch.empty(B, device=feats.device, dtype=torch.float32)
            loss = torch.empty((), device=feats.device, dtype=torch.float32)
            _lib.check(lib.se_head_linear_sisdr_f32(_lib.ptr(feats), _lib.ptr(w3), _lib.ptr(bias), _lib.ptr(lin), _lib.ptr(stats), B, F, D, N, act, _lib.ptr(predicted),
                                                    None, _lib.ptr(tarc), _lib.ptr(lens), int(len_div), float(ceps), scratch[2:].data_ptr(), _lib.ptr(loss_b),
                                                    scratch.data_ptr(), _lib.ptr(loss), _lib.stream()), 'se_head_linear_sisdr_f32')
            predicted._se_sisdr = (loss, predicted._version, tar, float(ceps))
        else:
            predicted = run(False)
        return predicted, {'offset': LazyTensor((B, F, N), feats.device, lambda: run(True))}

    def enhance_scored(self, features, linears, linear_tar, lengths, len_div, eps):
        if torch.is_grad_enabled() or torch.is_inference_mode_enabled() or not features.is_cuda or not getattr(self, 'lazy_offset', True):
            return self.forward(features, linears)
        return self._forward_lazy(features, linears, sisdr=(linear_tar, lengths, len_div, eps))


class SpecHead(nn.Module):

    def __init__(self, output_size, ckpt, activation='ReLU', random_init=False, eps=1e-6, **kwargs):
        super().__init__()
        assert ckpt != ''
        ckpt = load_checkpoint(ckpt) if isinstance(ckpt, str) else ckpt
        trans_config = TransformerConfig(ckpt['Settings']['Config'])
        trans_spechead = TransformerSpecPredictionHead(trans_config, output_size)
        trans_spechead.load_state_dict(ckpt['SpecHead'])
        assert trans_spechead.output.out_features == output_size
        self.spechead = trans_spechead
        self.eps = eps
        target_config = ckpt['Settings']['Config']['online']['target']
        self.log = False if 'log' not in target_config else target_config['log']
        self.activation = activation
        _act_id(activation)
        if random_init:
            for param in self.parameters():
                if param.dim() >= 2:
                    nn.init.xavier_uniform_(param.data)
                else:
                    nn.init.constant_(param.data, 0)

    def forward(self, features, **kwargs):
        sh = self.spechead
        if sh._needs_grad():
            from .spechead_train import SpecHeadTrainFn
            predicted, log_predicted = SpecHeadTrainFn.apply(features, sh.dense.weight, sh.dense.bias, sh.LayerNorm.weight, sh.LayerNorm.bias,
                                                             sh.output.weight, sh.output.bias, sh.LayerNorm.variance_epsilon, self.log,
                                                             _act_id(self.activation), self.eps)
            return predicted, {'log_predicted': log_predicted}
        predicted, log_predicted = sh._engine.spechead(sh, None, features, mode='full', log_target=self.log, act=self.activation, eps=self.eps)
        return predicted, {'log_predicted': log_predicted}


class Mockingjay(nn.Module):

    def __init__(self, dckpt, activation='ReLU', eps=1e-6, **kwargs):
        super().__init__()
        options = {'ckpt_file': dckpt, 'load_pretrain': 'True', 'no_grad': 'False', 'dropout': 'default', 'spec_aug': 'False',
                   'spec_aug_prev': 'True', 'weighted_sum': 'False', 'select_layer': -1, 'permute_input': 'False'}
        ckpt = load_checkpoint(dckpt)
        pretrain_config = ckpt['Settings']['Config']
        online = pretrain_config['online']
        def feat_dim(cfg):
            base = {'mel': online.get('n_mels', 40), 'linear': online.get('n_freq', 201), 'phase': online.get('n_freq', 201),
                    'complx': 2 * online.get('n_freq', 201)}[cfg['feat_type']]
            return base * (1 + int(cfg.get('delta', 0)))
        inp_dim, tar_dim = feat_dim(online['input']), feat_dim(online['target'])
        self.mockingjay = TRANSFORMER(options, inp_dim)
        trans_config = TransformerConfig(pretrain_config)
        trans_spechead = TransformerSpecPredictionHead(trans_config, tar_dim)
        trans_spechead.load_state_dict(ckpt['SpecHead'])
        assert trans_spechead.output.out_features == tar_dim
        self.spechead = trans_spechead
        self.eps = eps
        target_config = online['target']
        self.log = False if 'log' not in target_config else target_config['log']
        self.activation = activation
        _act_id(activation)

    def forward(self, features, **kwargs):
        features = self.mockingjay(features)
        sh = self.spechead
        if sh._needs_grad() or features.requires_grad:
            from .spechead_train import SpecHeadTrainFn
            predicted, log_predicted = SpecHeadTrainFn.apply(features, sh.dense.weight, sh.dense.bias, sh.LayerNorm.weight, sh.LayerNorm.bias,
                                                             sh.output.weight, sh.output.bias, sh.LayerNorm.variance_epsilon, self.log,
                                                             _act_id(self.activation), self.eps)
            return predicted, {'log_predicted': log_predicted}
        predicted, log_predicted = sh._engine.spechead(sh, None, features, mode='full', log_target=self.log, act=self.activation, eps=self.eps)
        return predicted, {'log_predicted': log_predicted}
```

speech-enhancement-by-s3prl_amd/objective.py:

```python
import torch
import torch.nn as nn

from . import _lib


_L1_SCRATCH = {}


def _l1_scratch(dev, B):
    key = (dev.index if dev.index is not None else torch.cuda.current_device(), torch.cuda.current_stream(dev).cuda_stream)
    n = int(_lib.load().se_l1_scratch_doubles(int(B)))
    t = _L1_SCRATCH.get(key)
    if t is None or t.numel() < n:
        t = _L1_SCRATCH[key] = torch.zeros(max(n, 1024), device=dev, dtype=torch.float64)
    return t


class _L1Fn(torch.autograd.Function):
    @staticmethod
    def forward(ctx, log_predicted, linear_tar, lengths, len_div, eps, reduce_fn):
        lib = _lib.load()
        lp = log_predicted.contiguous().float()
        tar = linear_tar.contiguous().float()
        B, F, K = lp.shape
        lens = lengths.to(device=lp.device, dtype=torch.int64).contiguous()
        sums = torch.empty(2, device=lp.device, dtype=torch.float64)
        need_grad = log_predicted.requires_grad
        grad = torch.empty_like(lp) if need_grad else None
        if reduce_fn is None:
            loss = torch.empty((), device=lp.device, dtype=torch.float32)
            rc = lib.se_l1_masked_loss_f32(_lib.ptr(lp), _lib.ptr(tar), _lib.ptr(lens), int(len_div), B, F, K, float(eps), _lib.ptr(_l1_scratch(lp.device, B)),
                                           _lib.ptr(sums), _lib.ptr(loss), _lib.ptr(grad), _lib.stream())
            if rc != 0:
                _L1_SCRATCH.clear()
            _lib.check(rc, 'se_l1_masked_loss_f32')
            ctx.save_for_backward(grad if grad is not None else torch.empty(0), sums)
            return loss
        if len_div:
            lens = lens // int(len_div) + 1
        _lib.check(lib.se_l1_masked_f32(_lib.ptr(lp), _lib.ptr(tar), _lib.ptr(lens), B, F, K, float(eps), _lib.ptr(sums),
                                        _lib.ptr(grad), _lib.stream()), 'se_l1_masked_f32')
        if reduce_fn is not None:
            sums = reduce_fn(sums)
        ctx.save_for_backward(grad if grad is not None else torch.empty(0), sums)
        return (sums[0] / sums[1]).float()

    @staticmethod
    def backward(ctx, g):
        sign, sums = ctx.saved_tensors
        return sign * (g / sums[1].float()), None, None, None, None, None


class L1(nn.Module):

    def __init__(self, eps=1e-10, **kwargs):
        super().__init__()
        self.eps = eps
        self.reduce_fn = None

    def forward(self, log_predicted, linear_tar, stft_length_masks=None, stft_lengths=None, wav_lengths=None, hop=None, **kwargs):
        if wav_lengths is not None and hop:
            loss = _L1Fn.apply(log_predicted, linear_tar, wav_lengths, int(hop), self.eps, self.reduce_fn)
            return loss, {}
        if stft_lengths is None:
            stft_lengths = stft_length_masks.sum(dim=-1)
        loss = _L1Fn.apply(log_predicted, linear_tar, stft_lengths, 0, self.eps, self.reduce_fn)
        return loss, {}


def _frame_lengths(stft_length_masks, stft_lengths, device):
    if stft_lengths is None:
        stft_lengths = stft_length_masks.sum(dim=-1)
    return stft_lengths.to(device=device, dtype=torch.int64).contiguous()


def sisdr_loss_inference(predicted, linear_tar, lengths, len_div, eps):
    lib = _lib.load()
    p, t = predicted.contiguous().float(), linear_tar.contiguous().float()
    B, F, N = p.shape
    lens = lengths.to(device=p.device, dtype=torch.int64).contiguous()
    scratch = torch.empty(int(lib.se_sisdr_spec_loss_scratch_doubles(B, F, N)) + 2, device=p.device, dtype=torch.float64)
    loss_b = torch.empty(B, device=p.device, dtype=torch.float32)
    loss = torch.empty((), device=p.device, dtype=torch.float32)
    _lib.check(lib.se_sisdr_spec_loss_f32(_lib.ptr(p), _lib.ptr(t), _lib.ptr(lens), int(len_div), B, F, N, float(eps), scratch[2:].data_ptr(), _lib.ptr(loss_b),
                                          scratch.data_ptr(), _lib.ptr(loss), _lib.stream()), 'se_sisdr_spec_loss_f32')
    return loss, loss_b


class _SISDRFn(torch.autograd.Function):
    @staticmethod
    def forward(ctx, predicted, linear_tar, lens, eps, reduce_fn):
        lib = _lib.load()
        p, t = predicted.contiguous().float(), linear_tar.contiguous().float()
        B, F, N = p.shape
        scratch = torch.empty(5 * B, device=p.device, dtype=torch.float64)
        loss_b = torch.empty(B, device=p.device, dtype=torch.float32)
        grad = torch.empty_like(p) if predicted.requires_grad else None
        _lib.check(lib.se_sisdr_spec_f32(_lib.ptr(p), _lib.ptr(t), _lib.ptr(lens), B, F, N, float(eps), 1.0, _lib.ptr(scratch), _lib.ptr(loss_b),
                                         _lib.ptr(grad), _lib.stream()), 'se_sisdr_spec_f32')
        sums = torch.stack([loss_b.double().sum(), torch.full((), float(B), device=p.device, dtype=torch.float64)])
        if reduce_fn is not None:
            sums = reduce_fn(sums)
        ctx.save_for_backward(grad if grad is not None else torch.empty(0), sums)
        return (sums[0] / sums[1]).float()

    @staticmethod
    def backward(ctx, g):
        grad, sums = ctx.saved_tensors
        return grad * (g / sums[1].float()), None, None, None, None


class SISDR(nn.Module):

    def __init__(self, eps=1e-10, **kwargs):
        super().__init__()
        self.eps = eps
        self.reduce_fn = None

    def forward(self, predicted, linear_tar, stft_length_masks=None, stft_lengths=None, wav_lengths=None, hop=None, **kwargs):
        no_grad = not (torch.is_grad_enabled() and predicted.requires_grad)
        if no_grad and self.reduce_fn is None and predicted.is_cuda:
            side = getattr(predicted, '_se_sisdr', None)
            if side is not None and side[1] == predicted._version and side[2] is linear_tar and side[3] == float(self.eps):
                return side[0], {}
            if wav_lengths is not None and hop:
                return sisdr_loss_inference(predicted, linear_tar, wav_lengths, int(hop), self.eps)[0], {}
            return sisdr_loss_inference(predicted, linear_tar, _frame_lengths(stft_length_masks, stft_lengths, predicted.device), 0, self.eps)[0], {}
        if stft_lengths is None and stft_length_masks is None and wav_lengths is not None and hop:
            stft_lengths = wav_lengths // int(hop) + 1
        lens = _frame_lengths(stft_length_masks, stft_lengths, predicted.device)
        return _SISDRFn.apply(predicted, linear_tar, lens, self.eps, self.reduce_fn), {}


class _WSDFn(torch.autograd.Function):
    @staticmethod
    def forward(ctx, linear_inp, offset, linear_tar, lens, alpha, db_interval, eps, reduce_fn, max_reduce_fn):
        lib = _lib.load()
        inp, off, tar = linear_inp.contiguous().float(), offset.contiguous().float(), linear_tar.contiguous().float()
        B, F, N = off.shape
        dev = off.device
        energy = torch.empty(B * F, device=dev, dtype=torch.float32)
        emax = torch.empty(1, device=dev, dtype=torch.float32)
        _lib.check(lib.se_wsd_energy_f32(_lib.ptr(tar), B, F, N, _lib.ptr(energy), _lib.ptr(emax), _lib.stream()), 'se_wsd_energy_f32')
        if max_reduce_fn is not None:
            emax = max_reduce_fn(emax)
        sums = torch.empty(3, device=dev, dtype=torch.float64)
        grad = torch.empty_like(off) if offset.requires_grad else None
        _lib.check(lib.se_wsd_f32(_lib.ptr(inp), _lib.ptr(off), _lib.ptr(tar), _lib.ptr(lens), _lib.ptr(energy), _lib.ptr(emax), B, F, N, float(alpha),
                                  float(db_interval), float(eps), 1.0, _lib.ptr(sums), _lib.ptr(grad), _lib.stream()), 'se_wsd_f32')
        tot = torch.stack([alpha * sums[0] + (1.0 - alpha) * sums[1], torch.full((), float(B), device=dev, dtype=torch.float64)])
        if reduce_fn is not None:
            tot = reduce_fn(tot)
        ctx.save_for_backward(grad if grad is not None else torch.empty(0), tot)
        return (tot[0] / tot[1]).float()

    @staticmethod
    def backward(ctx, g):
        grad, tot = ctx.saved_tensors
        return None, grad * (g / tot[1].float()), None, None, None, None, None, None, None


class WSD(nn.Module):

    def __init__(self, alpha=0.5, db_interval=30, eps=1e-10, **kwargs):
        super().__init__()
        self.alpha, self.db_interval, self.eps = alpha, db_interval, eps
        self.reduce_fn = None
# ... 190 lines not shown
```

speech-enhancement-by-s3prl_amd/pipeline.py:

```python
import copy

import torch

from . import decode
from .checkpoint import reference_paras
from .heads import SpecHead
from .objective import L1
from .preprocessor import OnlinePreprocessor
from .transformer import TRANSFORMER

PRETRAIN_SAMPLE = {
    'transformer': {'input_dim': 80, 'downsample_rate': 1, 'hidden_size': 768, 'num_hidden_layers': 6,
                    'num_attention_heads': 12, 'intermediate_size': 3072, 'hidden_act': 'gelu',
                    'hidden_dropout_prob': 0.1, 'attention_probs_dropout_prob': 0.1, 'initializer_range': 0.02,
                    'layer_norm_eps': '1e-12', 'share_layer': False},
    'online': {'sample_rate': 16000, 'max_time': 10000, 'target_level': -25, 'noise_proportion': 0.5, 'snrs': [3, 6],
               'win_ms': 25, 'hop_ms': 10, 'n_freq': 201, 'n_mels': 40, 'n_mfcc': 13,
               'input': {'feat_type': 'mel', 'channel': 0, 'log': True, 'delta': 1, 'cmvn': True},
               'target': {'feat_type': 'linear', 'channel': 1, 'log': True, 'delta': 0, 'cmvn': False}},
}
BASELINE_FEAT = {'feat_type': 'mel', 'log': True, 'delta': 2, 'cmvn': False}


def make_config(layers=6, hidden=768, heads=12, intermediate=3072):
    cfg = copy.deepcopy(PRETRAIN_SAMPLE)
    cfg['transformer'].update(num_hidden_layers=layers, hidden_size=hidden, num_attention_heads=heads, intermediate_size=intermediate)
    return cfg


def random_upstream_states(config, inp_dim=80, spec_out=201, seed=0):
    t = config['transformer']
    H, I, L, r = t['hidden_size'], t['intermediate_size'], t['num_hidden_layers'], float(t['initializer_range'])
    g = torch.Generator().manual_seed(seed)
    sd = {}

    def lin(d, name, o, i):
        d[name + '.weight'] = torch.randn(o, i, generator=g) * r
        d[name + '.bias'] = torch.randn(o, generator=g) * r

    def ln(d, name):
        d[name + '.weight'] = 1.0 + 0.1 * torch.randn(H, generator=g)
        d[name + '.bias'] = 0.1 * torch.randn(H, generator=g)

    lin(sd, 'input_representations.spec_transform', H, inp_dim)
    ln(sd, 'input_representations.LayerNorm')
    for i in range(L):
        p = f'encoder.layer.{i}.'
        for n in ('query', 'key', 'value'):
            lin(sd, p + 'attention.self.' + n, H, H)
        lin(sd, p + 'attention.output.dense', H, H)
        ln(sd, p + 'attention.output.LayerNorm')
        lin(sd, p + 'intermediate.dense', I, H)
        lin(sd, p + 'output.dense', H, I)
        ln(sd, p + 'output.LayerNorm')
    head = {}
    lin(head, 'dense', H, H)
    ln(head, 'LayerNorm')
    lin(head, 'output', spec_out, H)
    return sd, head


def synthetic_checkpoint(config=None, seed=0, inp_dim=80, spec_out=201):
    config = config or make_config()
    sd, head = random_upstream_states(config, inp_dim, spec_out, seed)
    return {'Settings': {'Config': config, 'Paras': reference_paras(downstream='SpecHead')}, 'Transformer': sd, 'SpecHead': head}


def build_upstream(ckpt, device):
    options = {'ckpt_file': '', 'load_pretrain': 'False', 'no_grad': 'True', 'dropout': 'default', 'spec_aug': 'False',
               'spec_aug_prev': 'True', 'weighted_sum': 'False', 'select_layer': -1, 'permute_input': 'False'}
    inp_dim = ckpt['Transformer']['input_representations.spec_transform.weight'].shape[1]
    out_dim = ckpt['SpecHead']['output.weight'].shape[0]
    upstream = TRANSFORMER(options, inp_dim, config=ckpt['Settings']['Config'])
    upstream.model.load_state_dict(ckpt['Transformer'])
    setattr(upstream, 'SpecHead', SpecHead(out_dim, ckpt))
    return upstream.to(device).eval()


def build_preprocessor(config, device, channel_inp=0, channel_tar=1, downstream_feat=None, upstream='transformer'):
    online = config['online']
    down = dict(downstream_feat or BASELINE_FEAT, channel=channel_inp)
    up = dict(online['input'], channel=channel_inp) if upstream == 'transformer' else dict(down)
    P = OnlinePreprocessor
    feat_list = [up, down, P.get_feat_config('linear', channel_inp), P.get_feat_config('phase', channel_inp),
                 P.get_feat_config('linear', channel_tar), P.get_feat_config('phase', channel_tar)]
    pre = OnlinePreprocessor(**online, feat_list=feat_list)
    pre.channel_inp, pre.channel_tar = channel_inp, channel_tar
    pre.encoder_side = upstream == 'transformer'
    return pre.to(device)


class UpstreamEnhanceStep:

    def __init__(self, preprocessor, upstream, criterion=None, streams=1):
        self.pre, self.up = preprocessor, upstream
        self.criterion = criterion or L1()
        self.streams = int(streams)
        self._side = None
        if self.streams > 1:
            self.up._engine.fused_ln_min_rows = 8192

    def _one(self, wavs, lengths, max_len, want_sums=False):
        feats_up, feats_down, lin_inp, ph_inp, lin_tar, ph_tar = self.pre(wavs)
        hidden = self.up(feats_up)
        predicted, res = self.up.SpecHead(hidden)
        wav_tar = wavs[:, self.pre.channel_tar, :]
        wav_pred = decode.decode_wav(self.pre, predicted, ph_inp, lengths, wav_tar, max_len=max_len)
        hop = self.pre._win_args['hop_length']
        if isinstance(self.criterion, L1):
            lens_kw = {'wav_lengths': lengths, 'hop': hop}
        else:
            lens_kw = {'stft_lengths': lengths // hop + 1}
        if want_sums:
            sums = []
            self.criterion.reduce_fn = lambda t: (sums.append(t) or t)
            try:
                self.criterion(log_predicted=res['log_predicted'], linear_tar=lin_tar, **lens_kw)
            finally:
                self.criterion.reduce_fn = None
            return wav_pred, sums[0], predicted
        loss, _ = self.criterion(log_predicted=res['log_predicted'], linear_tar=lin_tar, **lens_kw)
        return wav_pred, loss, predicted

    @torch.no_grad()
    def __call__(self, wavs, lengths, max_len=None):
        B = wavs.shape[0]
        if self.streams <= 1 or B < 2 * self.streams:
            return self._one(wavs, lengths, max_len)
        if max_len is None:
            max_len = int(lengths.max().item())
        dev = wavs.device
        if self._side is None:
            self._side = [torch.cuda.Stream(device=dev) for _ in range(self.streams)]
        cur = torch.cuda.current_stream(dev)
        bounds = [B * i // self.streams for i in range(self.streams + 1)]
        parts = []
        for i, st in enumerate(self._side):
            st.wait_stream(cur)
            with torch.cuda.stream(st):
                parts.append(self._one(wavs[bounds[i]:bounds[i + 1]], lengths[bounds[i]:bounds[i + 1]], max_len, want_sums=True))
        for st in self._side:
            cur.wait_stream(st)
        for p in parts:
            for t in p:
                t.record_stream(cur)
        wav_pred = torch.cat([p[0] for p in parts], dim=0)
        predicted = torch.cat([p[2] for p in parts], dim=0)
        sums = torch.stack([p[1] for p in parts]).sum(dim=0)
        return wav_pred, (sums[0] / sums[1]).float(), predicted


class HeadEnhanceStep:

    fuse_criterion = True

    def __init__(self, preprocessor, head, criterion=None):
        self.pre, self.head, self.criterion = preprocessor, head, criterion
        if getattr(head, 'cmvn', False) and hasattr(head, 'eps'):
            self.pre.head_stats_eps = float(head.eps)

    @torch.no_grad()
    def __call__(self, wavs, lengths, max_len=None):
        from .objective import SISDR
        feats_up, feats_down, lin_inp, ph_inp, lin_tar, ph_tar = self.pre(wavs)
        hop = self.pre._win_args['hop_length']
        if (self.fuse_criterion and isinstance(self.criterion, SISDR) and self.criterion.reduce_fn is None and hasattr(self.head, 'enhance_scored') and
                not lin_tar.is_inference()):
            predicted, res = self.head.enhance_scored(feats_down, lin_inp, lin_tar, lengths, hop, self.criterion.eps)
        else:
            predicted, res = self.head(features=feats_down, linears=lin_inp)
        wav_tar = wavs[:, self.pre.channel_tar, :]
        wav_pred = decode.decode_wav(self.pre, predicted, ph_inp, lengths, wav_tar, max_len=max_len)
        loss = None
        if self.criterion is not None:
            if isinstance(self.criterion, (L1, SISDR)):
                lens_kw = {'wav_lengths': lengths, 'hop': hop}
            else:
                lens_kw = {'stft_lengths': lengths // hop + 1}
            loss, _ = self.criterion(predicted=predicted, linear_inp=lin_inp, linear_tar=lin_tar, **lens_kw, **res)
        return wav_pred, predicted, lin_tar, loss


class MockingjayFinetuneStep:

    def __init__(self, preprocessor, model, optimizer, grad_clip=1.0):
        from .dist import DataParallelTrainStep
        self.pre, self.model = preprocessor, model
        self.criterion = L1()
        self.dp = DataParallelTrainStep(model, self.criterion, optimizer, grad_clip=grad_clip)

    def __call__(self, wavs, lengths):
        with torch.no_grad():
            feats_up, feats_down, lin_inp, ph_inp, lin_tar, ph_tar = self.pre(wavs)
        predicted, res = self.model(features=feats_up, linears=lin_inp)
        stft_lengths = lengths // self.pre._win_args['hop_length'] + 1
        loss, _ = self.criterion(log_predicted=res['log_predicted'], linear_tar=lin_tar, stft_lengths=stft_lengths)
        grad_norm, skipped = self.dp.step(loss)
        return loss.detach(), grad_norm, skipped


def build_mockingjay(ckpt, device, tmp_dir=None):
    import os
    import tempfile
    from .heads import Mockingjay
    d = tmp_dir or tempfile.mkdtemp(prefix='se_amd_ckpt_')
    path = os.path.join(d, 'states.ckpt')
    torch.save(ckpt, path)
    try:
        model = Mockingjay(path)
    finally:
        os.remove(path)
        if tmp_dir is None:
            os.rmdir(d)
    return model.to(device).train()


class GraphedStep:

    def __init__(self, fn, wavs, lengths, *static_args, warmup=3):
        self.fn, self.static_args = fn, static_args
        self.wavs = wavs.clone()
        self.lengths = lengths.clone()
        side = torch.cuda.Stream(device=wavs.device)
        side.wait_stream(torch.cuda.current_stream(wavs.device))
        with torch.cuda.stream(side):
            for _ in range(warmup):
                fn(self.wavs, self.lengths, *static_args)
        torch.cuda.current_stream(wavs.device).wait_stream(side)
        torch.cuda.synchronize(wavs.device)
        self.graph = torch.cuda.CUDAGraph()
        with torch.cuda.graph(self.graph):
            self.out = fn(self.wavs, self.lengths, *static_args)

    def __call__(self, wavs, lengths):
        self.wavs.copy_(wavs, non_blocking=True)
        self.lengths.copy_(lengths, non_blocking=True)
        self.graph.replay()
        return self.out


class HeadFinetuneStep:

    def __init__(self, preprocessor, head, optimizer, criterion=None, grad_clip=1.0):
        from .dist import DataParallelTrainStep
        self.pre, self.head = preprocessor, head
        self.criterion = criterion or L1()
        self.dp = DataParallelTrainStep(head, self.criterion, optimizer, grad_clip=grad_clip)

    def __call__(self, wavs, lengths):
        with torch.no_grad():
            feats_up, feats_down, lin_inp, ph_inp, lin_tar, ph_tar = self.pre(wavs)
        predicted, res = self.head(features=feats_down, linears=lin_inp)
        if getattr(self.criterion, 'wants_wav', False):
            wav_tar = wavs[:, getattr(self.pre, 'channel_tar', 1), :]
            wav_predicted = decode.decode_wav(self.pre, predicted, ph_inp, lengths, wav_tar)
            loss, _ = self.criterion(wav_predicted=wav_predicted, wav_tar=wav_tar, lengths=lengths)
        else:
            stft_lengths = lengths // self.pre._win_args['hop_length'] + 1
            loss, _ = self.criterion(predicted=predicted, linear_inp=lin_inp, linear_tar=lin_tar, stft_lengths=stft_lengths, **res)
        grad_norm, skipped = self.dp.step(loss)
        return loss.detach(), grad_norm, skipped
# ... 1 lines not shown
```

speech-enhancement-by-s3prl_amd/preprocessor.py:

```python
import torch
import torch.nn as nn

from . import _lib

N_SAMPLED_PSEUDO_WAV = 2


class LazyTensor(torch.Tensor):

    @staticmethod
    def __new__(cls, shape, device, materialize, *args, **kwargs):
        r = torch.Tensor._make_wrapper_subclass(cls, tuple(shape), dtype=torch.float32, device=device, requires_grad=False)
        r._materialize_fn, r._value = materialize, None
        return r

    def materialize(self):
        if self._value is None:
            self._value = self._materialize_fn()
            self._materialize_fn = None
        return self._value

    @classmethod
    def __torch_dispatch__(cls, func, types, args=(), kwargs=None):
        from torch.utils._pytree import tree_map
# ... 319 lines not shown
        F = T // self._win_args['hop_length'] + 1
        K = self._n_freq
        dev = wavs3.device
        with_phase = sorted(ch for ch, k in need.items() if 'phase' in k)
        ch_inp = getattr(self, 'channel_inp', None)
        if ch_inp not in with_phase:
            ch_inp = with_phase[0]
        chans = sorted(need)
        outs = {}
        for ch in chans:
            o = {}
            if 'linear' in need[ch]:
                o['linear'] = torch.empty(B, F, K, device=dev, dtype=torch.float32)
            if 'mel' in need[ch]:
                o['mel'] = torch.empty(B, self._n_mels, F, device=dev, dtype=torch.float32)
            if ch == ch_inp and 'phase' in need[ch]:
                o['_tphase'] = torch.empty(B, F, K, device=dev, dtype=torch.int32)
            outs[ch] = o
        g = lambda o, k: _lib.ptr(o.get(k))
        a = chans[0]
        b = chans[1] if len(chans) > 1 else -1
        ob = outs[b] if b >= 0 else {}
        _lib.check(lib.se_stft_tphase_f32(self._plan(dev), _lib.ptr(wavs3), B, C, T, a, g(outs[a], 'linear'), g(outs[a], '_tphase'), g(outs[a], 'mel'),
                                          b, g(ob, 'linear'), g(ob, '_tphase'), g(ob, 'mel'), _lib.stream()), 'se_stft_tphase_f32')
        if wavs3.is_inference():
            wavs3 = wavs3.clone()
            ver0 = None
        else:
            ver0 = wavs3._version
        for ch in chans:
            if 'phase' in need[ch]:
                def materialize(ch=ch):
                    if ver0 is not None and wavs3._version != ver0:
                        raise RuntimeError('LazyPhase: the waveform batch this phase belongs to was modified in place after preprocessor(wavs) returned '
                                           '(version %d -> %d); read the phase before re-using the input buffer, or set preprocessor.lazy_phase = False'
                                           % (ver0, wavs3._version))
                    return self._stft_channel(wavs3, ch, {'phase'})['phase'].reshape(*lead, F, K)
                ph = outs[ch].get('_tphase')
                outs[ch]['phase'] = LazyPhase((*lead, F, K), dev, materialize, None if ph is None else ph.reshape(*lead, F, K))
        return outs

    ENCODER_IN_PAD = 128

    def _select(self, raw, raw_time_major, log, delta, cmvn, encoder_side=False):
        lib = _lib.load()
        if raw_time_major:
            B, F, D = raw.shape
        else:
            B, D, F = raw.shape
        Dout = D * (1 + delta)
        out = torch.empty(B, F, Dout, device=raw.device, dtype=torch.float32)
        side = encoder_side and Dout <= self.ENCODER_IN_PAD
        xin = torch.empty(B * F, self.ENCODER_IN_PAD, device=raw.device, dtype=torch.bfloat16) if side else None
        valid = torch.empty(B, device=raw.device, dtype=torch.int32) if side else None
        if not self.one_pass_features:
            nbytes = lib.se_features_workspace_bytes(B, D, F, delta)
            ws = torch.empty(nbytes, device=raw.device, dtype=torch.uint8)
            _lib.check(lib.se_features2_f32(_lib.ptr(raw), int(raw_time_major), B, D, F, int(bool(log)), int(delta),
                                            int(bool(cmvn)), float(self.eps), _lib.ptr(out), _lib.ptr(ws), nbytes,
                                            _lib.ptr(xin), self.ENCODER_IN_PAD if side else 0, _lib.ptr(valid), _lib.stream()), 'se_features2_f32')
        else:
            hs_eps = None if (cmvn or encoder_side) else self.head_stats_eps
            nbytes = (lib.se_features3_workspace_bytes(B, D, delta) if cmvn else
                      lib.se_features3_colstats_workspace_bytes(B, D, F, delta) if hs_eps is not None else 0)
            ws = torch.empty(nbytes, device=raw.device, dtype=torch.uint8) if nbytes else None
            colstats = torch.empty(B, Dout, 2, device=raw.device, dtype=torch.float32) if hs_eps is not None else None
            _lib.check(lib.se_features3_f32(_lib.ptr(raw), int(raw_time_major), B, D, F, int(bool(log)), int(delta), int(bool(cmvn)), float(self.eps),
                                            _lib.ptr(out), _lib.ptr(ws), nbytes, _lib.ptr(xin), self.ENCODER_IN_PAD if side else 0, _lib.ptr(valid),
                                            _lib.ptr(colstats), float(hs_eps) if hs_eps is not None else 0.0, _lib.stream()), 'se_features3_f32')
            if colstats is not None:
                out._se_colstats = (colstats, float(hs_eps))
        if side:
            out._se_side = (xin, valid)
        return out

    one_pass_features = True
    head_stats_eps = None

    def forward(self, wavs=None, feat_list=None):
        feat_list = self._check_list(feat_list)
        if wavs is None:
            max_channel_id = max(int(a['channel']) if 'channel' in a else 0 for a in feat_list)
            wavs = self._pseudo_wavs[0].view(1, 1, -1).repeat(1, max_channel_id + 1, 1)
        assert wavs.dim() >= 3
        wavs, home = self._stage(wavs)
        wavs = wavs.contiguous().float()
        lead = wavs.shape[:-2]
        wavs3 = wavs.reshape(-1, wavs.shape[-2], wavs.shape[-1])

        need, mfcc_channels = {}, set()
        for a in feat_list:
            ft = a['feat_type']
            if ft == 'mfcc':
                mfcc_channels.add(int(a.get('channel', 0)))
                continue
            need.setdefault(int(a.get('channel', 0)), set()).add(ft)
        lazy = self._tphase_path_ok(need, wavs3, home)
        if lazy:
            planes = self._stft_tphase(wavs3, need, lead)
        elif len(need) == 2:
            planes = self._stft_two_channels(wavs3, need)
        else:
            planes = {ch: self._stft_channel(wavs3, ch, kinds) for ch, kinds in need.items()}
        for ch in mfcc_channels:
            planes.setdefault(ch, {})['mfcc'] = self._mfcc_channel(wavs3, ch)

        feats = []
        done = {}
        for a in feat_list:
            ft, ch = a['feat_type'], int(a.get('channel', 0))
            log, delta, cmvn = bool(a.get('log', False)), int(a.get('delta', 0)), bool(a.get('cmvn', False))
            key = (ft, ch, log, delta, cmvn)
            if key in done:
                feats.append(done[key])
                continue
            raw = planes[ch][ft]
            if type(raw) is LazyPhase:
                feats.append(raw)
                continue
            first = len(feats) == 0 and home == wavs3.device and getattr(self, 'encoder_side', True)
            time_major = ft != 'mel'
            if (ft == 'mel' or log or delta or cmvn) and lazy and len(feats) > 0 and getattr(self, 'lazy_features', True):
                Bp, Dp, Fp = (raw.shape[0], raw.shape[2], raw.shape[1]) if time_major else raw.shape
                feat = LazyTensor((*lead, Fp, Dp * (1 + delta)), home,
                                  lambda raw=raw, tm=time_major, a=(log, delta, cmvn): self._select(raw, tm, *a).reshape(*lead, Fp_(raw, tm), -1))
                done[key] = feat
                feats.append(feat)
                continue
            if ft == 'mel':
                feat = self._select(raw, False, log, delta, cmvn, encoder_side=first)
            elif log or delta or cmvn:
                feat = self._select(raw, True, log, delta, cmvn, encoder_side=first)
            else:
                feat = raw
            side = getattr(feat, '_se_side', None)
            cst = getattr(feat, '_se_colstats', None)
            feat = feat.reshape(*lead, *feat.shape[-2:]).to(home)
            if side is not None:
                if not feat.is_inference():
                    feat._se_side = side + (feat._version,)
            if cst is not None and feat.is_cuda and not feat.is_inference():
                feat._se_colstats = cst + (feat._version,)
            done[key] = feat
            feats.append(feat)
        return feats

    def istft(self, linears=None, phases=None, linear_power=2, complxs=None):
        if complxs is not None:
            raise NotImplementedError('istft(complxs=) is unused by the reference (runner.py:267 passes linears, phases)')
        assert linears is not None and phases is not None
        wav, _ = self.istft_with_sumsq(linears, phases, linear_power=linear_power)
        return wav

    def istft_with_sumsq(self, linears, phases, linear_power=2, lengths=None, out_len=None, ref=None):
        if torch.is_grad_enabled() and linears.requires_grad:
            if float(linear_power) != 2.0:
                raise NotImplementedError('the iSTFT is differentiated for linear_power = 2 only')
            if not linears.is_cuda:
                raise _lib.SEError('the iSTFT backward takes device tensors only; there is no CPU fallback')
            return _IstftFn.apply(linears, self, phases, lengths, out_len, ref)[:2 if ref is None else 3]
        linears, home = self._stage(linears)
        if (type(phases) is LazyPhase and phases._tphase is not None and phases._value is None and float(linear_power) == 2.0 and
                phases._tphase.device == linears.device and home == linears.device):
            return self._istft_tphase(linears, phases._tphase, lengths, out_len, ref=ref)
        phases = phases.to(linears.device)
        lib = _lib.load()
        lead = linears.shape[:-2]
        F, K = linears.shape[-2:]
        lin = linears.contiguous().float().reshape(-1, F, K)
        ph = phases.contiguous().float().reshape(-1, F, K)
        B = lin.shape[0]
        n_out = self._win_args['hop_length'] * (F - 1)
        stride = n_out if out_len is None else max(int(out_len), n_out)
        wav = torch.empty(B, stride, device=lin.device, dtype=torch.float32)
        sumsq = None
        if lengths is not None:
            lengths = lengths.to(device=lin.device, dtype=torch.int64).contiguous()
            sumsq = torch.empty(B, device=lin.device, dtype=torch.float32)
        _lib.check(lib.se_istft_f32(self._plan(lin.device), _lib.ptr(lin), _lib.ptr(ph), B, F, float(linear_power),
                                    _lib.ptr(wav), stride, _lib.ptr(lengths), _lib.ptr(sumsq), _lib.stream()), 'se_istft_f32')
        if ref is not None:
            return wav.reshape(*lead, stride).to(home), (None if sumsq is None else sumsq.to(home)), None
        return wav.reshape(*lead, stride).to(home), (None if sumsq is None else sumsq.to(home))

    def _istft_tphase(self, linears, tphase, lengths, out_len, log_input=False, ref=None):
        if log_input and torch.is_grad_enabled() and linears.requires_grad:
            raise NotImplementedError('the iSTFT of a log-power plane (log_input) is not differentiated')
        lib = _lib.load()
        lead = linears.shape[:-2]
        F, K = linears.shape[-2:]
        lin = linears.contiguous().float().reshape(-1, F, K)
        ph = tphase.reshape(-1, F, K)
        assert ph.shape[0] == lin.shape[0] and ph.is_contiguous()
        B = lin.shape[0]
        n_out = self._win_args['hop_length'] * (F - 1)
        stride = n_out if out_len is None else max(int(out_len), n_out)
        wav = torch.empty(B, stride, device=lin.device, dtype=torch.float32)
        sums = None
        use_ref = (ref is not None and lengths is not None and ref.dim() == 2 and ref.shape[0] == B and ref.dtype == torch.float32 and ref.is_cuda and
                   ref.stride(1) == 1 and ref.shape[1] >= stride)
        if lengths is not None:
            lengths = lengths.to(device=lin.device, dtype=torch.int64).contiguous()
            sums = torch.empty(2 if use_ref else 1, B, device=lin.device, dtype=torch.float32)
        _lib.check(lib.se_istft_tphase_f32(self._plan(lin.device), _lib.ptr(lin), _lib.ptr(ph), B, F, int(bool(log_input)), _lib.ptr(wav), stride,
                                           _lib.ptr(lengths), None if sums is None else sums[0].data_ptr(),
                                           ref.data_ptr() if use_ref else None, int(ref.stride(0)) if use_ref else 0,
                                           sums[1].data_ptr() if use_ref else None, _lib.stream()), 'se_istft_tphase_f32')
        wav = wav.reshape(*lead, stride)
        if ref is None:
            return wav, (None if sums is None else sums[0])
        return wav, (None if sums is None else sums[0]), (sums[1] if use_ref else None)

    def _stft(self, wav2d, window=None):
        wav2d, home = self._stage(wav2d)
        out = self._stft_channel(wav2d.contiguous().float().unsqueeze(1), 0, {'complx'})['complx']
        N, F, _ = out.shape
        return out.view(N, F, self._n_freq, 2).permute(0, 2, 1, 3).contiguous().to(home)

    @staticmethod
    def _magphase(complx, power=2.0):
        mag = complx.pow(2).sum(-1).pow(power / 2.0)
        phase = torch.atan2(complx[..., 1], complx[..., 0])
        return mag, phase
```

speech-enhancement-by-s3prl_amd/transformer.py:

```python
import ctypes
import warnings

import numpy as np
import weakref

import os

import torch
import torch.nn as nn

from . import _lib
from .checkpoint import load_checkpoint
from .preprocessor import OnlinePreprocessor


class TransformerConfig(object):

    def __init__(self, config):
        t = config['transformer']
        self.downsample_rate = int(t.get('downsample_rate', 1))
        self.hidden_size = int(t.get('hidden_size', 768))
        self.num_hidden_layers = int(t.get('num_hidden_layers', 6))
        self.num_attention_heads = int(t.get('num_attention_heads', 12))
        self.hidden_act = t.get('hidden_act', 'gelu')
# ... 470 lines not shown
                       'se_gemm_res_ln_bf16')
            _lib.check(lib.se_split3_bf16(_lib.ptr(dst), H, M, H, H, 0, _lib.ptr(x3), _lib.stream()), 'se_split3_bf16')

        ln3(x, ir.LayerNorm, xa)
        x = xa
        for layer in model.encoder.layer:
            att = layer.attention
            qb = torch.cat([att.self.query.bias.detach(), att.self.key.bias.detach(), att.self.value.bias.detach()]).float().contiguous()
            wq, _ = self._w3((att.self.query.weight, att.self.key.weight, att.self.value.weight))
            gemm3(x3, 3 * H, wq, qb, 3 * H, out=qkv)
            _lib.check(lib.se_mhsa_fwd_x3_split_f32(_lib.ptr(qkv), _lib.ptr(lengths), B, T, heads, _lib.ptr(c3), H, _lib.stream()), 'se_mhsa_fwd_x3_split_f32')
            wo, _ = self._w3(att.output.dense.weight)
            xn = xb if x is xa else xa
            if rowln & 1:
                gemm_ln3(c3, 3 * H, wo, w(att.output.dense.bias), x, att.output.LayerNorm, xn)
            else:
                gemm3(c3, 3 * H, wo, w(att.output.dense.bias), H, residual=x, out=a)
                ln3(a, att.output.LayerNorm, xn)
            x = xn
            w1, _ = self._w3(layer.intermediate.dense.weight)
            _lib.check(lib.se_gemm_x3out_bf16(_lib.ptr(x3), 3 * H, _lib.ptr(w1), 3 * H, _lib.ptr(w(layer.intermediate.dense.bias)), M, I, 3 * H,
                                              _lib.SE_ACT['GELU'], _lib.ptr(h3), I, _lib.stream()), 'se_gemm_x3out_bf16')
            w2, _ = self._w3(layer.output.dense.weight)
            xn = xb if x is xa else xa
            if rowln & 2:
                gemm_ln3(h3, 3 * I, w2, w(layer.output.dense.bias), x, layer.output.LayerNorm, xn)
            else:
                gemm3(h3, 3 * I, w2, w(layer.output.dense.bias), H, residual=x, out=a)
                ln3(a, layer.output.LayerNorm, xn)
            x = xn
        return x.view(B, T, H)

    def _encode_x3_unchained(self, model, x, ir, lengths, B, T, H, heads, I, M):
        lib = _lib.load()
        dev = x.device
        w = lambda p: p.detach().contiguous()
        x = self._ln32(x, ir.LayerNorm, M, H)
        qkv = torch.empty(M, 3 * H, device=dev, dtype=torch.float32)
        ctx = torch.empty(M, H, device=dev, dtype=torch.float32)
        for layer in model.encoder.layer:
            att = layer.attention
            qb = torch.cat([att.self.query.bias.detach(), att.self.key.bias.detach(), att.self.value.bias.detach()]).float().contiguous()
            self._linear3(x, (att.self.query.weight, att.self.key.weight, att.self.value.weight), qb, M, 3 * H, H, out=qkv)
            _lib.check(lib.se_mhsa_fwd_x3_f32(_lib.ptr(qkv), _lib.ptr(lengths), B, T, heads, _lib.ptr(ctx), _lib.stream()), 'se_mhsa_fwd_x3_f32')
            a = self._linear3(ctx, att.output.dense.weight, w(att.output.dense.bias), M, H, H, residual=x)
            x = self._ln32(a, att.output.LayerNorm, M, H)
            h = self._linear3(x, layer.intermediate.dense.weight, w(layer.intermediate.dense.bias), M, I, H, act=_lib.SE_ACT['GELU'])
            o = self._linear3(h, layer.output.dense.weight, w(layer.output.dense.bias), M, H, I, residual=x)
            x = self._ln32(o, layer.output.LayerNorm, M, H)
        return x.view(B, T, H)

    def spechead_x3(self, head, hidden, mode='raw', log_target=False, act='ReLU', eps=1e-6):
        if not hidden.is_cuda:
            raise _lib.SEError('TransformerSpecPredictionHead runs on MI355X only (no CPU fallback)')
        lib = _lib.load()
        hidden = hidden.contiguous().float()
        B, T, H = hidden.shape
        M, N = B * T, head.output.out_features
        w = lambda p: p.detach().contiguous()
        h = self._linear3(hidden.view(M, H), head.dense.weight, w(head.dense.bias), M, H, H, act=_lib.SE_ACT['GELU'])
        h = self._ln32(h, head.LayerNorm, M, H)
        raw = self._linear3(h, head.output.weight, w(head.output.bias), M, N, H).view(B, T, N)
        if mode == 'raw':
            return raw
        pred, logp = torch.empty_like(raw), torch.empty_like(raw)
        _lib.check(lib.se_spec_epilogue_f32(_lib.ptr(raw), raw.numel(), int(bool(log_target)), _lib.SE_ACT[act], float(eps), _lib.ptr(pred), _lib.ptr(logp),
                                            _lib.stream()), 'se_spec_epilogue_f32')
        return pred, logp

    def spechead_fp32(self, head, hidden, mode='raw', log_target=False, act='ReLU', eps=1e-6):
        if not hidden.is_cuda:
            raise _lib.SEError('TransformerSpecPredictionHead runs on MI355X only (no CPU fallback)')
        lib = _lib.load()
        hidden = hidden.contiguous().float()
        B, T, H = hidden.shape
        M, N = B * T, head.output.out_features
        w = lambda p: p.detach().contiguous()
        h = self._gemm32(hidden.view(M, H), w(head.dense.weight), w(head.dense.bias), M, H, H, act=_lib.SE_ACT['GELU'])
        h = self._ln32(h, head.LayerNorm, M, H)
        raw = self._gemm32(h, w(head.output.weight), w(head.output.bias), M, N, H).view(B, T, N)
        if mode == 'raw':
            return raw
        pred, logp = torch.empty_like(raw), torch.empty_like(raw)
        _lib.check(lib.se_spec_epilogue_f32(_lib.ptr(raw), raw.numel(), int(bool(log_target)), _lib.SE_ACT[act], float(eps), _lib.ptr(pred), _lib.ptr(logp),
                                            _lib.stream()), 'se_spec_epilogue_f32')
        return pred, logp

    def encode(self, model, head, feats, lengths=None):
        if self.precision == 'fp32':
            return self.encode_fp32(model, feats, lengths)
        if self.precision == 'bf16x3':
            return self.encode_x3(model, feats, lengths)
        if not feats.is_cuda:
            raise _lib.SEError('TRANSFORMER runs on MI355X only (no CPU fallback): move the module and inputs to the GPU')
        lib = _lib.load()
        side = getattr(feats, '_se_side', None)
        feats_c = feats.contiguous().float()
        xin = None
        if side is not None and feats_c is feats and side[2] == feats._version and side[0].shape[0] == feats.shape[0] * feats.shape[1]:
            xin = side[0]
            if lengths is None:
                lengths = side[1]
        feats = feats_c
        B, T, D = feats.shape
        h = self._ensure(model, head, feats.device)
        ws, n = self._workspace(h, B, T, feats.device)
        if lengths is None:
            lengths = torch.empty(B, device=feats.device, dtype=torch.int32)
            _lib.check(lib.se_valid_lengths_i32(_lib.ptr(feats), B, T, D, _lib.ptr(lengths), _lib.stream()), 'se_valid_lengths_i32')
        H_ = model.config.hidden_size
        hidden = torch.empty(B, T, H_, device=feats.device, dtype=torch.float32)
        _lib.check(lib.se_encoder_fwd2_bf16(h, _lib.ptr(feats), _lib.ptr(xin), _lib.ptr(lengths), B, T, _lib.ptr(hidden), _lib.ptr(ws), n,
                                            _lib.stream()), 'se_encoder_fwd2_bf16')
        if not hidden.is_inference():
            _LAST_ENCODE[(feats.device.index, torch.cuda.current_stream(feats.device).cuda_stream)] = (weakref.ref(hidden), hidden._version, B, T, H_, ws)
        return hidden

    @staticmethod
    def _cached_workspace(hidden, B, T, H, n):
        e = _LAST_ENCODE.get((hidden.device.index, torch.cuda.current_stream(hidden.device).cuda_stream))
        if e is not None and e[0]() is hidden and e[1:5] == (hidden._version, B, T, H) and e[5].numel() >= n:
            return e[5], 1
        return None, 0

    def spechead(self, head, model, hidden, mode='raw', log_target=False, act='ReLU', eps=1e-6):
        if self.precision == 'fp32':
            return self.spechead_fp32(head, hidden, mode=mode, log_target=log_target, act=act, eps=eps)
        if self.precision == 'bf16x3':
            return self.spechead_x3(head, hidden, mode=mode, log_target=log_target, act=act, eps=eps)
        if not hidden.is_cuda:
            raise _lib.SEError('TransformerSpecPredictionHead runs on MI355X only (no CPU fallback)')
        lib = _lib.load()
        hidden = hidden.contiguous().float()
        B, T, H = hidden.shape
        h = self._ensure(model, head, hidden.device)
        ws, n = self._workspace(h, B, T, hidden.device)
        cws, cached = self._cached_workspace(hidden, B, T, H, n)
        if cached:
            ws = cws
        N = head.output.out_features
        dev = hidden.device
        if mode == 'raw':
            raw = torch.empty(B, T, N, device=dev, dtype=torch.float32)
            _lib.check(lib.se_spechead_fwd2_bf16(h, _lib.ptr(hidden), B, T, 0, 0, float(eps), None, None, _lib.ptr(raw), _lib.ptr(ws), n,
                                                 cached, _lib.stream()), 'se_spechead_fwd2_bf16')
            return raw
        pred = torch.empty(B, T, N, device=dev, dtype=torch.float32)
        logp = torch.empty(B, T, N, device=dev, dtype=torch.float32)
        _lib.check(lib.se_spechead_fwd2_bf16(h, _lib.ptr(hidden), B, T, int(bool(log_target)), _lib.SE_ACT[act], float(eps),
                                             _lib.ptr(pred), _lib.ptr(logp), None, _lib.ptr(ws), n, cached,
                                             _lib.stream()), 'se_spechead_fwd2_bf16')
        return pred, logp


_LAST_ENCODE = {}


def _str2bool(v):
    return v if isinstance(v, bool) else str(v) == 'True'


class TRANSFORMER(nn.Module):

    def __init__(self, options, inp_dim, config=None, online_config=None):
        super().__init__()
        if config is not None:
            self.all_states = None
            self.config = config
        else:
            self.all_states = load_checkpoint(options['ckpt_file'])
            self.config = self.all_states['Settings']['Config']
        self.no_grad = _str2bool(options.get('no_grad', 'False'))
        self.spec_aug = _str2bool(options.get('spec_aug', 'False'))
        self.weighted_sum = _str2bool(options.get('weighted_sum', 'False'))
        self.select_layer = int(options.get('select_layer', -1))
        self.permute_input = _str2bool(options.get('permute_input', 'False'))
        if self.weighted_sum or self.select_layer != -1:
            raise NotImplementedError('weighted_sum / select_layer != -1 are unused by the reference (model.py:138-139)')
        if self.spec_aug:
            raise NotImplementedError("spec_aug is 'False' at every reference call site (model.py:136)")
        if options.get('dropout', 'default') != 'default':
            d = float(options['dropout'])
            self.config['transformer']['hidden_dropout_prob'] = d
            self.config['transformer']['attention_probs_dropout_prob'] = d
        self.model_config = TransformerConfig(self.config)
        self.dr = self.model_config.downsample_rate
        if self.dr != 1:
            raise NotImplementedError('downsample_rate != 1 (config/pretrain_sample.yaml:3 uses 1)')
        self.hidden_size = self.model_config.hidden_size
        self.num_layers = self.model_config.num_hidden_layers
        if online_config is None and 'online' in self.config:
            online_config = self.config['online']
        if online_config is not None:
            self.preprocessor = OnlinePreprocessor(**online_config)
            self.preprocessor.feat_list = [online_config['input']] if 'input' in online_config else None
        self.inp_dim = inp_dim
        self.model = TransformerModel(self.model_config, inp_dim)
        if _str2bool(options.get('load_pretrain', 'False')) and self.all_states is not None:
            self.model.load_state_dict(self.all_states['Transformer'])
        self.out_dim = self.hidden_size
        self._engine = _Engine()
        self._warned = False
        self.all_states = None

    def set_precision(self, precision):
        assert precision in ('bf16', 'fp32', 'bf16x3')
        self._engine.precision = precision
        sh = getattr(self, 'SpecHead', None)
        if sh is not None and hasattr(sh, 'spechead'):
            sh.spechead.set_precision(precision)
        return self

    def forward(self, x):
        train = torch.is_grad_enabled() and not self.no_grad and any(p.requires_grad for p in self.model.parameters())
        if train and self._engine.precision != 'bf16':
            raise NotImplementedError("precisions 'fp32' / 'bf16x3' are the inference parity modes; training runs the bf16 kernels")
        dropout_p = self.model_config.hidden_dropout_prob if self.training else 0.0
        if dropout_p > 0:
            if self.model_config.attention_probs_dropout_prob != dropout_p:
                raise NotImplementedError('hidden_dropout_prob != attention_probs_dropout_prob (config/pretrain_sample.yaml:9-10 sets both to 0.1)')
            if not train and not self._warned:
                warnings.warn('TRANSFORMER in train() mode without gradients: the fused inference path runs, dropout is not applied')
                self._warned = True
        if self.permute_input:
            x = x.permute(1, 0, 2)
        if hasattr(self, 'preprocessor') and x.size(-1) != self.inp_dim:
            x = self.preprocessor(x.transpose(1, 2).contiguous())[0]
        if train:
            seed = int(torch.randint(0, 2 ** 62, (1,)).item()) if dropout_p > 0 else 0
            self.last_dropout = (dropout_p, seed)
            out = self._engine.encode_train(self.model, x, dropout_p=dropout_p, seed=seed)
        else:
            with torch.no_grad():
                out = self._engine.encode(self.model, None, x)
        if self.permute_input:
            out = out.permute(1, 0, 2)
        return out


class dummy_upstream(nn.Module):

    def __init__(self, input_dim):
        super().__init__()
        self.out_dim = input_dim

    def forward(self, features):
        return features
```

Before: 8586 utt/s.

## Fuse spec-head epilogue with masked L1 loss and pre-clear iSTFT sums

Adds a fused tail kernel that applies the spec-head activation and log, writes predicted and log-predicted, and accumulates the masked L1 loss against the log target. The final sum uses a last-block reduction, and the same kernel zeroes the iSTFT sum-of-squares buffer so the iSTFT can skip its separate memset. This removes the separate epilogue kernel, the separate L1 loss pass over the prediction and a zero-fill launch. In exchange it adds a cross-workgroup atomic and ticket scheme with persistent scratch state, and the loss is only fused for plain L1 criteria.

```diff
diff --git a/include/se_amd.h b/include/se_amd.h
--- a/include/se_amd.h
+++ b/include/se_amd.h
@@ -72,6 +72,9 @@
 int se_istft_tphase_f32(const se_plan* plan, const float* power, const unsigned* tphase, int B, int F, int log_input,
                         float* wav_out, int wav_stride, const int64_t* lengths, float* sumsq_out,
                         const float* ref, int ref_stride, float* ref_sumsq_out, void* stream);
+int se_istft_tphase_acc_f32(const se_plan* plan, const float* power, const unsigned* tphase, int B, int F, int log_input,
+                            float* wav_out, int wav_stride, const int64_t* lengths, float* sumsq_out,
+                            const float* ref, int ref_stride, float* ref_sumsq_out, int sums_cleared, void* stream);
 
 int se_masked_sumsq_f32(const float* x, int B, int T, int x_stride, const int64_t* lengths, float* sums, void* stream);
 
@@ -161,6 +164,14 @@
 int se_spechead_fwd2_bf16(const se_encoder* enc, const float* hidden, int B, int T, int log_target, int act, float eps,
                           float* predicted, float* log_predicted, float* raw,
                           void* workspace, size_t workspace_bytes, int x_bf_valid, void* stream);
+size_t se_spec_tail_l1_scratch_doubles(void);
+int se_spec_tail_l1_f32(const float* p, int M, int N, int ld, int F, int log_target, int act, float eps, float* predicted, float* log_predicted,
+                        const float* linear_tar, const int64_t* lengths, int len_div, float l1_eps, double* scratch, double* sums_out,
+                        float* loss_out, void* clear, size_t clear_bytes, void* stream);
+int se_spechead_fwd_l1_bf16(const se_encoder* enc, const float* hidden, int B, int T, int log_target, int act, float eps,
+                            float* predicted, float* log_predicted, void* workspace, size_t workspace_bytes, int x_bf_valid,
+                            const float* linear_tar, const int64_t* lengths, int len_div, float l1_eps, double* scratch,
+                            double* sums_out, float* loss_out, void* clear, size_t clear_bytes, void* stream);
 
 int se_valid_lengths_i32(const float* feats, int B, int T, int D, int32_t* lengths, void* stream);
 
diff --git a/speech-enhancement-by-s3prl_amd/_lib.py b/speech-enhancement-by-s3prl_amd/_lib.py
--- a/speech-enhancement-by-s3prl_amd/_lib.py
+++ b/speech-enhancement-by-s3prl_amd/_lib.py
@@ -59,6 +59,7 @@
     'se_stft2_f32': (c_int, [_P, _P, c_int, c_int, c_int, c_int, _P, _P, _P, _P, c_int, _P, _P, _P, _P, _P]),
     'se_stft_tphase_f32': (c_int, [_P, _P, c_int, c_int, c_int, c_int, _P, _P, _P, c_int, _P, _P, _P, _P]),
     'se_istft_tphase_f32': (c_int, [_P, _P, _P, c_int, c_int, c_int, _P, c_int, _P, _P, _P, c_int, _P, _P]),
+    'se_istft_tphase_acc_f32': (c_int, [_P, _P, _P, c_int, c_int, c_int, _P, c_int, _P, _P, _P, c_int, _P, c_int, _P]),
     'se_features_workspace_bytes': (c_size_t, [c_int, c_int, c_int, c_int]),
     'se_features_f32': (c_int, [_P, c_int, c_int, c_int, c_int, c_int, c_int, c_int, c_float, _P, _P, c_size_t, _P]),
     'se_features2_f32': (c_int, [_P, c_int, c_int, c_int, c_int, c_int, c_int, c_int, c_float, _P, _P, c_size_t, _P, c_int, _P, _P]),
@@ -97,6 +98,10 @@
     'se_encoder_fwd2_bf16': (c_int, [_P, _P, _P, _P, c_int, c_int, _P, _P, c_size_t, _P]),
     'se_spechead_fwd_bf16': (c_int, [_P, _P, c_int, c_int, c_int, c_int, c_float, _P, _P, _P, _P, c_size_t, _P]),
     'se_spechead_fwd2_bf16': (c_int, [_P, _P, c_int, c_int, c_int, c_int, c_float, _P, _P, _P, _P, c_size_t, c_int, _P]),
+    'se_spec_tail_l1_scratch_doubles': (c_size_t, []),
+    'se_spec_tail_l1_f32': (c_int, [_P, c_int, c_int, c_int, c_int, c_int, c_int, c_float, _P, _P, _P, _P, c_int, c_float, _P, _P, _P, _P, c_size_t, _P]),
+    'se_spechead_fwd_l1_bf16': (c_int, [_P, _P, c_int, c_int, c_int, c_int, c_float, _P, _P, _P, c_size_t, c_int, _P, _P, c_int, c_float, _P, _P, _P, _P,
+                                        c_size_t, _P]),
     'se_valid_lengths_i32': (c_int, [_P, c_int, c_int, c_int, _P, _P]),
     'se_gemm_bf16': (c_int, [_P, c_int, _P, c_int, _P, _P, c_int, c_int, c_int, c_int, _P, _P, c_int, _P]),
     'se_gemm_res_ln_bf16': (c_int, [_P, c_int, _P, c_int, _P, _P, _P, _P, c_float, c_int, c_int, c_int, _P, _P, _P]),
diff --git a/speech-enhancement-by-s3prl_amd/csrc/encoder.hip b/speech-enhancement-by-s3prl_amd/csrc/encoder.hip
--- a/speech-enhancement-by-s3prl_amd/csrc/encoder.hip
+++ b/speech-enhancement-by-s3prl_amd/csrc/encoder.hip
@@ -221,6 +221,92 @@
       if (predicted) predicted[o] = pred;
       if (log_predicted) log_predicted[o] = lp;
     }
+  }
+}
+
+constexpr int kTailRows = 4;
+
+__global__ __launch_bounds__(256) void spec_tail_l1_kernel(const float* __restrict__ p, int M, int N, int ld, int F, int log_target, int act, float eps,
+                                                           float* __restrict__ predicted, float* __restrict__ log_predicted,
+                                                           const float* __restrict__ linear_tar, const int64_t* __restrict__ lengths, int len_div,
+                                                           float l1_eps, double* __restrict__ scratch, double* __restrict__ out,
+                                                           float* __restrict__ loss, uint32_t* __restrict__ clear, int n_clear) {
+  __shared__ float red[4];
+  __shared__ int s_last;
+  __shared__ double dred[2][4];
+  if (blockIdx.x == 0)
+    for (int i = threadIdx.x; i < n_clear; i += 256) clear[i] = 0u;
+  float s = 0.f;
+  for (int c = threadIdx.x; c < N; c += 256) {
+    for (int r0 = blockIdx.x; r0 < M; r0 += kTailRows * gridDim.x) {
+      float v[kTailRows], lt[kTailRows];
+      bool ok[kTailRows];
+#pragma unroll
+      for (int j = 0; j < kTailRows; ++j) {
+        const int r = r0 + j * gridDim.x;
+        const bool in = r < M;
+        const int rr = in ? r : 0;
+        const int b = rr / F, f = rr - b * F;
+        const int wl = (int)min(max(lengths[b], (int64_t)0), (int64_t)0x7fffffff);
+        ok[j] = in && f < (len_div > 0 ? wl / len_div + 1 : wl);
+        v[j] = in ? p[(size_t)r * ld + c] : 0.f;
+        lt[j] = ok[j] ? linear_tar[(size_t)r * N + c] : 1.f;
+      }
+#pragma unroll
+      for (int j = 0; j < kTailRows; ++j) {
+        const int r = r0 + j * gridDim.x;
+        if (r < M) {
+          float pred, lp;
+          if (log_target) {
+            pred = expf(v[j]);
+            lp = v[j];
+          } else {
+            pred = v[j];
+            lp = logf(v[j] + eps);
+          }
+          if (act == SE_ACT_RELU) pred = fmaxf(pred, 0.f);
+          else if (act == SE_ACT_SIGMOID) pred = 1.f / (1.f + expf(-pred));
+          const size_t o = (size_t)r * N + c;
+          predicted[o] = pred;
+          log_predicted[o] = lp;
+          if (ok[j]) s += fabsf(lp - logf(lt[j] + l1_eps));
+        }
+      }
+    }
+  }
+#pragma unroll
+  for (int off = 32; off > 0; off >>= 1) s += __shfl_down(s, off);
+  if ((threadIdx.x & 63) == 0) red[threadIdx.x >> 6] = s;
+  __syncthreads();
+  if (threadIdx.x == 0) {
+    const double part = (double)red[0] + (double)red[1] + (double)red[2] + (double)red[3];
+    __hip_atomic_store(&scratch[2 + blockIdx.x], part, __ATOMIC_RELAXED, __HIP_MEMORY_SCOPE_AGENT);
+    asm volatile("s_waitcnt vmcnt(0)" ::: "memory");
+    s_last = atomicAdd(reinterpret_cast<unsigned long long*>(scratch), 1ull) == (unsigned long long)gridDim.x - 1;
+  }
+  __syncthreads();
+  if (!s_last) return;
+  __builtin_amdgcn_fence(__ATOMIC_ACQUIRE, "agent");
+  double acc = 0.0, cnt = 0.0;
+  for (int i = threadIdx.x; i < (int)gridDim.x; i += 256) acc += __hip_atomic_load(&scratch[2 + i], __ATOMIC_RELAXED, __HIP_MEMORY_SCOPE_AGENT);
+  for (int b = threadIdx.x; b < M / F; b += 256) {
+    const int wl = (int)min(max(lengths[b], (int64_t)0), (int64_t)0x7fffffff);
+    cnt += (double)min(F, len_div > 0 ? wl / len_div + 1 : wl) * (double)N;
+  }
+#pragma unroll
+  for (int off = 32; off > 0; off >>= 1) {
+    acc += __shfl_down(acc, off);
+    cnt += __shfl_down(cnt, off);
+  }
+  if ((threadIdx.x & 63) == 0) { dred[0][threadIdx.x >> 6] = acc; dred[1][threadIdx.x >> 6] = cnt; }
+  __syncthreads();
+  if (threadIdx.x == 0) {
+    const double sum = (dred[0][0] + dred[0][1]) + (dred[0][2] + dred[0][3]);
+    const double n = (dred[1][0] + dred[1][1]) + (dred[1][2] + dred[1][3]);
+    out[0] = sum;
+    out[1] = n;
+    *loss = (float)(sum / n);
+    __hip_atomic_store(reinterpret_cast<unsigned long long*>(scratch), 0ull, __ATOMIC_RELAXED, __HIP_MEMORY_SCOPE_AGENT);
   }
 }
 
@@ -326,6 +412,36 @@
   SE_REQUIRE(p && n > 0 && (predicted || log_predicted), "se_spec_epilogue_f32: bad argument");
   const int grid = (int)std::min<size_t>((n + 255) / 256, 8192);
   hipLaunchKernelGGL(se::spec_epilogue_kernel, dim3(grid), dim3(256), 0, se::as_stream(stream), p, n, log_target, act, eps, predicted, log_predicted);
+  SE_LAUNCH_CHECK();
+  return SE_OK;
+}
+
+namespace se {
+constexpr int kTailMaxWgs = 8192;
+static int tail_wgs(int M) {
+  static int env = -1;
+  if (env < 0) {
+    const char* e = getenv("SE_AMD_TAIL_WGS");
+    env = e ? std::max(1, std::min(atoi(e), kTailMaxWgs)) : 0;
+  }
+  return std::min(M, env ? env : 1024);
+}
+}
+
+extern "C" size_t se_spec_tail_l1_scratch_doubles(void) { return 2 + (size_t)se::kTailMaxWgs; }
+
+extern "C" int se_spec_tail_l1_f32(const float* p, int M, int N, int ld, int F, int log_target, int act, float eps, float* predicted,
+                                   float* log_predicted, const float* linear_tar, const int64_t* lengths, int len_div, float l1_eps,
+                                   double* scratch, double* sums_out, float* loss_out, void* clear, size_t clear_bytes, void* stream) {
+  SE_REQUIRE(p && predicted && log_predicted && linear_tar && lengths && scratch && sums_out && loss_out, "se_spec_tail_l1_f32: null argument");
+  SE_REQUIRE(M > 0 && N > 0 && ld >= N && F > 0 && M % F == 0 && len_div >= 0, "se_spec_tail_l1_f32: bad shape M=%d N=%d ld=%d F=%d", M, N, ld, F);
+  SE_REQUIRE(act == SE_ACT_IDENTITY || act == SE_ACT_RELU || act == SE_ACT_SIGMOID, "se_spec_tail_l1_f32: activation must be Identity, ReLU or Sigmoid");
+  SE_REQUIRE((clear == nullptr) == (clear_bytes == 0) && (reinterpret_cast<uintptr_t>(clear) & 3) == 0 && (clear_bytes & 3) == 0 &&
+                 clear_bytes <= ((size_t)1 << 20),
+             "se_spec_tail_l1_f32: `clear` must be 4-byte aligned words, at most 1 MiB");
+  hipLaunchKernelGGL(se::spec_tail_l1_kernel, dim3(se::tail_wgs(M)), dim3(256), 0, se::as_stream(stream), p, M, N, ld, F, log_target ? 1 : 0, act, eps,
+                     predicted, log_predicted, linear_tar, lengths, len_div, l1_eps, scratch, sums_out, loss_out, reinterpret_cast<uint32_t*>(clear),
+                     (int)(clear_bytes / 4));
   SE_LAUNCH_CHECK();
   return SE_OK;
 }
@@ -635,9 +751,23 @@
   return se_spechead_fwd2_bf16(enc, hidden, B, T, log_target, act, eps, predicted, log_predicted, raw, workspace, workspace_bytes, 0, stream);
 }
 
-extern "C" int se_spechead_fwd2_bf16(const se_encoder* enc, const float* hidden, int B, int T, int log_target, int act, float eps,
-                                     float* predicted, float* log_predicted, float* raw,
-                                     void* workspace, size_t workspace_bytes, int x_bf_valid, void* stream) {
+namespace se {
+struct SpecTailL1 {
+  const float* linear_tar;
+  const int64_t* lengths;
+  int len_div;
+  float l1_eps;
+  double* scratch;
+  double* sums_out;
+  float* loss_out;
+  void* clear;
+  size_t clear_bytes;
+};
+}
+
+static int spechead_fwd(const se_encoder* enc, const float* hidden, int B, int T, int log_target, int act, float eps,
+                        float* predicted, float* log_predicted, float* raw,
+                        void* workspace, size_t workspace_bytes, int x_bf_valid, const se::SpecTailL1* tail, void* stream) {
   SE_REQUIRE(enc && hidden && workspace && (predicted || log_predicted || raw), "se_spechead_fwd_bf16: null argument");
   SE_REQUIRE(enc->cfg.spec_out > 0, "se_spechead_fwd_bf16: encoder was created without a spec head");
   SE_REQUIRE(B > 0 && T > 0, "se_spechead_fwd_bf16: bad shape");
@@ -670,6 +800,9 @@
   const int ldp = raw ? N : (N + 7) & ~7;
   SE_REQUIRE(ldp <= H, "se_spechead_fwd_bf16: spec_out %d exceeds the hidden size %d", N, H);
   if ((rc = se_gemm_bf16(w.ctx, H, enc->sh_out_w, H, enc->sh_out_b, nullptr, M, Np, H, SE_ACT_IDENTITY, nullptr, p, ldp, stream))) return rc;
+  if (tail)
+    return se_spec_tail_l1_f32(p, M, N, ldp, T, log_target, act, eps, predicted, log_predicted, tail->linear_tar, tail->lengths, tail->len_div,
+                               tail->l1_eps, tail->scratch, tail->sums_out, tail->loss_out, tail->clear, tail->clear_bytes, stream);
   if (predicted || log_predicted) {
     hipLaunchKernelGGL(se::spec_epilogue_rows_kernel, dim3(std::min(M, 8192)), dim3(256), 0, st, p, M, N, ldp, log_target, act, eps, predicted,
                        log_predicted);
@@ -677,3 +810,18 @@
   }
   return SE_OK;
 }
+
+extern "C" int se_spechead_fwd2_bf16(const se_encoder* enc, const float* hidden, int B, int T, int log_target, int act, float eps,
+                                     float* predicted, float* log_predicted, float* raw,
+                                     void* workspace, size_t workspace_bytes, int x_bf_valid, void* stream) {
+  return spechead_fwd(enc, hidden, B, T, log_target, act, eps, predicted, log_predicted, raw, workspace, workspace_bytes, x_bf_valid, nullptr, stream);
+}
+
+extern "C" int se_spechead_fwd_l1_bf16(const se_encoder* enc, const float* hidden, int B, int T, int log_target, int act, float eps,
+                                       float* predicted, float* log_predicted, void* workspace, size_t workspace_bytes, int x_bf_valid,
+                                       const float* linear_tar, const int64_t* lengths, int len_div, float l1_eps, double* scratch,
+                                       double* sums_out, float* loss_out, void* clear, size_t clear_bytes, void* stream) {
+  SE_REQUIRE(predicted && log_predicted, "se_spechead_fwd_l1_bf16: null argument");
+  const se::SpecTailL1 tail = {linear_tar, lengths, len_div, l1_eps, scratch, sums_out, loss_out, clear, clear_bytes};
+  return spechead_fwd(enc, hidden, B, T, log_target, act, eps, predicted, log_predicted, nullptr, workspace, workspace_bytes, x_bf_valid, &tail, stream);
+}
diff --git a/speech-enhancement-by-s3prl_amd/csrc/istft.hip b/speech-enhancement-by-s3prl_amd/csrc/istft.hip
--- a/speech-enhancement-by-s3prl_amd/csrc/istft.hip
+++ b/speech-enhancement-by-s3prl_amd/csrc/istft.hip
@@ -324,6 +324,12 @@
 extern "C" int se_istft_tphase_f32(const se_plan* plan, const float* power, const unsigned* tphase, int B, int F, int log_input,
                                    float* wav_out, int wav_stride, const int64_t* lengths, float* sumsq_out,
                                    const float* ref, int ref_stride, float* ref_sumsq_out, void* stream) {
+  return se_istft_tphase_acc_f32(plan, power, tphase, B, F, log_input, wav_out, wav_stride, lengths, sumsq_out, ref, ref_stride, ref_sumsq_out, 0, stream);
+}
+
+extern "C" int se_istft_tphase_acc_f32(const se_plan* plan, const float* power, const unsigned* tphase, int B, int F, int log_input,
+                                       float* wav_out, int wav_stride, const int64_t* lengths, float* sumsq_out,
+                                       const float* ref, int ref_stride, float* ref_sumsq_out, int sums_cleared, void* stream) {
   SE_REQUIRE(plan && power && tphase && wav_out, "se_istft_tphase_f32: null argument");
   SE_REQUIRE(B > 0 && B <= 65535 && F >= 2, "se_istft_tphase_f32: bad B=%d F=%d", B, F);
   const int n_out = plan->geom.hop * (F - 1);
@@ -344,7 +350,7 @@
     if (rc == SE_OK && ref_sumsq_out) rc = se_masked_sumsq_f32(ref, B, std::min(wav_stride, ref_stride), ref_stride, lengths, ref_sumsq_out, stream);
     return rc;
   }
-  if (sumsq_out) {
+  if (sumsq_out && !sums_cleared) {
     int zrc_;
     if (ref_sumsq_out == sumsq_out + B) zrc_ = se::zero_async(sumsq_out, sizeof(float) * 2 * B, st);
     else {
diff --git a/speech-enhancement-by-s3prl_amd/decode.py b/speech-enhancement-by-s3prl_amd/decode.py
--- a/speech-enhancement-by-s3prl_amd/decode.py
+++ b/speech-enhancement-by-s3prl_amd/decode.py
@@ -91,12 +91,12 @@
     return audio
 
 
-def decode_wav(preprocessor, linear, phase, lengths, target_level=-25, max_len=None):
+def decode_wav(preprocessor, linear, phase, lengths, target_level=-25, max_len=None, cleared_sums=None):
     if max_len is None:
         max_len = int(lengths.max().item())
     ref = target_level if isinstance(target_level, torch.Tensor) and target_level.dim() == 2 else None
     if ref is not None:
-        wav, sumsq, ref_sumsq = preprocessor.istft_with_sumsq(linear, phase, lengths=lengths, out_len=max_len, ref=ref)
+        wav, sumsq, ref_sumsq = preprocessor.istft_with_sumsq(linear, phase, lengths=lengths, out_len=max_len, ref=ref, cleared_sums=cleared_sums)
         return masked_normalize_decibel(wav, target_level, lengths, audio_sumsq=sumsq, inplace=True, ref_sumsq=ref_sumsq)
     wav, sumsq = preprocessor.istft_with_sumsq(linear, phase, lengths=lengths, out_len=max_len)
     return masked_normalize_decibel(wav, target_level, lengths, audio_sumsq=sumsq, inplace=True)
diff --git a/speech-enhancement-by-s3prl_amd/heads.py b/speech-enhancement-by-s3prl_amd/heads.py
--- a/speech-enhancement-by-s3prl_amd/heads.py
+++ b/speech-enhancement-by-s3prl_amd/heads.py
@@ -195,6 +195,18 @@
         predicted, log_predicted = sh._engine.spechead(sh, None, features, mode='full', log_target=self.log, act=self.activation, eps=self.eps)
         return predicted, {'log_predicted': log_predicted}
 
+    def can_score_l1(self, features, linear_tar, lengths):
+        return (not self.spechead._needs_grad() and self.spechead._engine.precision == 'bf16' and features.is_cuda and
+                torch.is_tensor(linear_tar) and linear_tar.is_cuda and linear_tar.dtype == torch.float32 and linear_tar.is_contiguous() and
+                linear_tar.shape[:2] == features.shape[:2] and linear_tar.shape[2] == self.spechead.output.out_features and
+                lengths.is_cuda and lengths.dtype == torch.int64 and lengths.is_contiguous())
+
+    def forward_scored_l1(self, features, linear_tar, lengths, len_div, l1_eps, clear=None):
+        sh = self.spechead
+        predicted, log_predicted, loss, sums = sh._engine.spechead_l1(sh, None, features, linear_tar, lengths, len_div, l1_eps, log_target=self.log,
+                                                                      act=self.activation, eps=self.eps, clear=clear)
+        return predicted, {'log_predicted': log_predicted}, loss, sums
+
 
 class Mockingjay(nn.Module):
 
diff --git a/speech-enhancement-by-s3prl_amd/objective.py b/speech-enhancement-by-s3prl_amd/objective.py
--- a/speech-enhancement-by-s3prl_amd/objective.py
+++ b/speech-enhancement-by-s3prl_amd/objective.py
@@ -13,6 +13,20 @@
     t = _L1_SCRATCH.get(key)
     if t is None or t.numel() < n:
         t = _L1_SCRATCH[key] = torch.zeros(max(n, 1024), device=dev, dtype=torch.float64)
+    return t
+
+
+_TAIL_SCRATCH = {}
+
+
+def _tail_scratch(dev, drop=False):
+    key = (dev.index if dev.index is not None else torch.cuda.current_device(), torch.cuda.current_stream(dev).cuda_stream)
+    if drop:
+        _TAIL_SCRATCH.pop(key, None)
+        return None
+    t = _TAIL_SCRATCH.get(key)
+    if t is None:
+        t = _TAIL_SCRATCH[key] = torch.zeros(int(_lib.load().se_spec_tail_l1_scratch_doubles()), device=dev, dtype=torch.float64)
     return t
 
 
diff --git a/speech-enhancement-by-s3prl_amd/pipeline.py b/speech-enhancement-by-s3prl_amd/pipeline.py
--- a/speech-enhancement-by-s3prl_amd/pipeline.py
+++ b/speech-enhancement-by-s3prl_amd/pipeline.py
@@ -100,13 +100,22 @@
         if self.streams > 1:
             self.up._engine.fused_ln_min_rows = 8192
 
+    fuse_tail = True
+
     def _one(self, wavs, lengths, max_len, want_sums=False):
         feats_up, feats_down, lin_inp, ph_inp, lin_tar, ph_tar = self.pre(wavs)
         hidden = self.up(feats_up)
-        predicted, res = self.up.SpecHead(hidden)
+        hop = self.pre._win_args['hop_length']
         wav_tar = wavs[:, self.pre.channel_tar, :]
+        head = self.up.SpecHead
+        if (self.fuse_tail and type(self.criterion) is L1 and self.criterion.reduce_fn is None and hasattr(head, 'forward_scored_l1') and
+                head.can_score_l1(hidden, lin_tar, lengths)):
+            sq = torch.empty(2, wavs.shape[0], device=wavs.device, dtype=torch.float32)
+            predicted, res, loss, sums = head.forward_scored_l1(hidden, lin_tar, lengths, hop, self.criterion.eps, clear=sq)
+            wav_pred = decode.decode_wav(self.pre, predicted, ph_inp, lengths, wav_tar, max_len=max_len, cleared_sums=sq)
+            return wav_pred, (sums if want_sums else loss), predicted
+        predicted, res = head(hidden)
         wav_pred = decode.decode_wav(self.pre, predicted, ph_inp, lengths, wav_tar, max_len=max_len)
-        hop = self.pre._win_args['hop_length']
         if isinstance(self.criterion, L1):
             lens_kw = {'wav_lengths': lengths, 'hop': hop}
         else:
diff --git a/speech-enhancement-by-s3prl_amd/preprocessor.py b/speech-enhancement-by-s3prl_amd/preprocessor.py
--- a/speech-enhancement-by-s3prl_amd/preprocessor.py
+++ b/speech-enhancement-by-s3prl_amd/preprocessor.py
@@ -495,7 +495,7 @@
         wav, _ = self.istft_with_sumsq(linears, phases, linear_power=linear_power)
         return wav
 
-    def istft_with_sumsq(self, linears, phases, linear_power=2, lengths=None, out_len=None, ref=None):
+    def istft_with_sumsq(self, linears, phases, linear_power=2, lengths=None, out_len=None, ref=None, cleared_sums=None):
         if torch.is_grad_enabled() and linears.requires_grad:
             if float(linear_power) != 2.0:
                 raise NotImplementedError('the iSTFT is differentiated for linear_power = 2 only')
@@ -505,7 +505,7 @@
         linears, home = self._stage(linears)
         if (type(phases) is LazyPhase and phases._tphase is not None and phases._value is None and float(linear_power) == 2.0 and
                 phases._tphase.device == linears.device and home == linears.device):
-            return self._istft_tphase(linears, phases._tphase, lengths, out_len, ref=ref)
+            return self._istft_tphase(linears, phases._tphase, lengths, out_len, ref=ref, cleared_sums=cleared_sums)
         phases = phases.to(linears.device)
         lib = _lib.load()
         lead = linears.shape[:-2]
@@ -526,7 +526,7 @@
             return wav.reshape(*lead, stride).to(home), (None if sumsq is None else sumsq.to(home)), None
         return wav.reshape(*lead, stride).to(home), (None if sumsq is None else sumsq.to(home))
 
-    def _istft_tphase(self, linears, tphase, lengths, out_len, log_input=False, ref=None):
+    def _istft_tphase(self, linears, tphase, lengths, out_len, log_input=False, ref=None, cleared_sums=None):
         if log_input and torch.is_grad_enabled() and linears.requires_grad:
             raise NotImplementedError('the iSTFT of a log-power plane (log_input) is not differentiated')
         lib = _lib.load()
@@ -545,10 +545,14 @@
         if lengths is not None:
             lengths = lengths.to(device=lin.device, dtype=torch.int64).contiguous()
             sums = torch.empty(2 if use_ref else 1, B, device=lin.device, dtype=torch.float32)
-        _lib.check(lib.se_istft_tphase_f32(self._plan(lin.device), _lib.ptr(lin), _lib.ptr(ph), B, F, int(bool(log_input)), _lib.ptr(wav), stride,
-                                           _lib.ptr(lengths), None if sums is None else sums[0].data_ptr(),
-                                           ref.data_ptr() if use_ref else None, int(ref.stride(0)) if use_ref else 0,
-                                           sums[1].data_ptr() if use_ref else None, _lib.stream()), 'se_istft_tphase_f32')
+        cleared = (sums is not None and use_ref and not log_input and cleared_sums is not None and cleared_sums.shape == sums.shape and
+                   cleared_sums.dtype == sums.dtype and cleared_sums.device == sums.device and cleared_sums.is_contiguous())
+        if cleared:
+            sums = cleared_sums
+        _lib.check(lib.se_istft_tphase_acc_f32(self._plan(lin.device), _lib.ptr(lin), _lib.ptr(ph), B, F, int(bool(log_input)), _lib.ptr(wav), stride,
+                                               _lib.ptr(lengths), None if sums is None else sums[0].data_ptr(),
+                                               ref.data_ptr() if use_ref else None, int(ref.stride(0)) if use_ref else 0,
+                                               sums[1].data_ptr() if use_ref else None, int(cleared), _lib.stream()), 'se_istft_tphase_acc_f32')
         wav = wav.reshape(*lead, stride)
         if ref is None:
             return wav, (None if sums is None else sums[0])
diff --git a/speech-enhancement-by-s3prl_amd/transformer.py b/speech-enhancement-by-s3prl_amd/transformer.py
--- a/speech-enhancement-by-s3prl_amd/transformer.py
+++ b/speech-enhancement-by-s3prl_amd/transformer.py
@@ -646,6 +646,33 @@
                                              _lib.stream()), 'se_spechead_fwd2_bf16')
         return pred, logp
 
+    def spechead_l1(self, head, model, hidden, linear_tar, lengths, len_div, l1_eps, log_target=False, act='ReLU', eps=1e-6, clear=None):
+        from .objective import _tail_scratch
+        assert self.precision == 'bf16' and hidden.is_cuda
+        lib = _lib.load()
+        hidden = hidden.contiguous().float()
+        B, T, H = hidden.shape
+        h = self._ensure(model, head, hidden.device)
+        ws, n = self._workspace(h, B, T, hidden.device)
+        cws, cached = self._cached_workspace(hidden, B, T, H, n)
+        if cached:
+            ws = cws
+        N = head.output.out_features
+        dev = hidden.device
+        assert linear_tar.shape == (B, T, N) and linear_tar.dtype == torch.float32 and lengths.dtype == torch.int64 and lengths.shape == (B,)
+        pred = torch.empty(B, T, N, device=dev, dtype=torch.float32)
+        logp = torch.empty(B, T, N, device=dev, dtype=torch.float32)
+        sums = torch.empty(2, device=dev, dtype=torch.float64)
+        loss = torch.empty((), device=dev, dtype=torch.float32)
+        rc = lib.se_spechead_fwd_l1_bf16(h, _lib.ptr(hidden), B, T, int(bool(log_target)), _lib.SE_ACT[act], float(eps), _lib.ptr(pred), _lib.ptr(logp),
+                                         _lib.ptr(ws), n, cached, _lib.ptr(linear_tar), _lib.ptr(lengths), int(len_div), float(l1_eps),
+                                         _lib.ptr(_tail_scratch(dev)), _lib.ptr(sums), _lib.ptr(loss), _lib.ptr(clear),
+                                         0 if clear is None else clear.numel() * clear.element_size(), _lib.stream())
+        if rc != 0:
+            _tail_scratch(dev, drop=True)
+        _lib.check(rc, 'se_spechead_fwd_l1_bf16')
+        return pred, logp, loss, sums
+
 
 _LAST_ENCODE = {}
 
```

After: 8589 utt/s (median of 3 runs). No clear change (+0.0%).
